# williamleif/GraphSAGE

Hardware: NVIDIA H100
Metric: seed_nodes_per_sec (higher is better)
Workload: dtype f32

## Files before the change

### graphsage_b200/_lib.py

```python
import ctypes
import os

import torch

_HERE = os.path.dirname(os.path.abspath(__file__))
LIB_PATH = os.path.join(_HERE, "csrc", "libgraphsage_b200.so")

ABI_VERSION = 2
GS_F32, GS_BF16, GS_F64 = 0, 1, 2
ACT_NONE, ACT_RELU = 0, 1
COMBINE_ADD, COMBINE_CONCAT = 0, 1
MATH_FP32_SIMT, MATH_TF32X3, MATH_TF32, MATH_BF16 = 0, 1, 2, 3
CSR_MEAN, CSR_MEAN_SELF, CSR_MAX = 0, 1, 2
MAX_SEGMENTS = 4

c_i32, c_i64, c_u64, c_vp = ctypes.c_int32, ctypes.c_int64, ctypes.c_uint64, ctypes.c_void_p


class Segment(ctypes.Structure):
    _fields_ = [("self_ids", c_vp), ("neigh_ids", c_vp), ("self_row0", c_i64), ("neigh_row0", c_i64),
                ("n", c_i64), ("k", c_i32), ("_pad", c_i32), ("out_row0", c_i64)]


MAX_SHARDS = 16


class ShardedTable(ctypes.Structure):
    _fields_ = [("base", c_vp * MAX_SHARDS), ("row_start", c_i64 * (MAX_SHARDS + 1)), ("n_shards", c_i32),
                ("my_shard", c_i32), ("n_global_rows", c_i64), ("zero_row", c_i64), ("remap", c_vp)]


class GemmPart(ctypes.Structure):
    _fields_ = [("A", c_vp), ("lda", c_i64), ("K", c_i32), ("B", c_vp), ("ldb", c_i64), ("N", c_i32)]


class RowRange(ctypes.Structure):
    _fields_ = [("ids", c_vp), ("row0", c_i64), ("n", c_i64)]


class GemmRowIds(ctypes.Structure):
    _fields_ = [("n_table_rows", c_i64), ("n_ranges", c_i32), ("_pad", c_i32), ("ranges", RowRange * MAX_SEGMENTS)]


MAX_EMBED_LISTS = 8
MAX_UNIQUE_SAMPLED = 1024
UNIQUE_DRAW_BUDGET = 1 << 20
WALK_MAX_WALKS = 1 << 20
WALK_MAX_LEN = 33


class EmbedGradList(ctypes.Structure):
    _fields_ = [("ids", c_vp), ("grad", c_vp), ("ldg", c_i64), ("n", c_i64), ("group", c_i32), ("scale", ctypes.c_float)]


class DropoutSite(ctypes.Structure):
    _fields_ = [("seed", c_u64), ("call", ctypes.c_uint32), ("rate", ctypes.c_float), ("call_dev", c_vp)]


_SIGNATURES = {
    "gs_version": (c_i32, []),
    "gs_last_error_string": (ctypes.c_char_p, []),
    "gs_set_tuning": (c_i32, [ctypes.c_char_p, c_i32]),
    "gs_sample_padded": (c_i32, [c_vp, c_i64, c_i32, c_vp, c_i64, c_i32, c_vp, c_u64, c_u64, c_vp, c_vp, c_vp]),
    "gs_sample_padded_khop": (c_i32, [c_vp, c_i64, c_i32, c_vp, c_i64, ctypes.POINTER(c_i32), c_i32, c_u64, c_u64, c_vp,
                                      ctypes.POINTER(c_vp), c_vp]),
    "gs_build_padded_adj": (c_i32, [c_vp, c_vp, c_i64, c_i32, c_vp, c_u64, c_u64, c_vp, c_vp, c_vp]),
    "gs_sample_unigram": (c_i32, [c_vp, c_i64, c_i32, c_u64, c_u64, c_vp, c_vp, c_vp]),
    "gs_sample_unigram_unique": (c_i32, [c_vp, c_i64, c_i32, c_u64, c_u64, c_vp, c_vp, c_vp, c_vp]),
    "gs_sample_csr": (c_i32, [c_vp, c_vp, c_i64, c_vp, c_i64, c_i32, c_i32, c_u64, c_u64, c_vp, c_i32, c_vp, c_vp]),
    "gs_perm_prefix_host": (c_i32, [c_u64, c_u64, c_i32, c_i32, ctypes.POINTER(c_i32)]),
    "gs_gather_rows": (c_i32, [c_vp, c_i32, c_i64, c_i32, c_i64, c_vp, c_i64, c_vp, c_i64, c_vp]),
    "gs_gather_mean": (c_i32, [c_vp, c_i32, c_i64, c_i32, c_i64, ctypes.POINTER(Segment), c_i32, c_i32, c_vp, c_vp,
                               c_i64, c_vp]),
    "gs_gather_mean_sharded": (c_i32, [ctypes.POINTER(ShardedTable), c_i32, c_i32, c_i64, ctypes.POINTER(Segment), c_i32,
                                       c_i32, c_i32, c_vp, c_vp, c_vp, c_i64, c_vp]),
    "gs_halo_begin": (c_i32, [c_vp, c_i64, c_vp, c_vp]),
    "gs_halo_claim": (c_i32, [ctypes.POINTER(ShardedTable), c_vp, c_i64, c_vp, c_vp, c_vp, c_i64, c_vp]),
    "gs_halo_fetch": (c_i32, [ctypes.POINTER(ShardedTable), c_i32, c_i64, c_vp, c_vp, c_i64, c_vp, c_i64, c_vp]),
    "gs_halo_translate": (c_i32, [ctypes.POINTER(ShardedTable), c_vp, c_i64, c_vp, c_vp, c_vp]),
    "gs_translate_ids": (c_i32, [ctypes.POINTER(ShardedTable), c_vp, c_i64, c_vp, c_vp]),
    "gs_gather_rows_sharded": (c_i32, [ctypes.POINTER(ShardedTable), c_i32, c_i32, c_i64, c_vp, c_i64, c_vp, c_i64, c_vp]),
    "gs_shard_alloc": (c_i32, [c_i64, ctypes.POINTER(c_vp)]),
    "gs_shard_free": (c_i32, [c_vp]),
    "gs_ipc_export": (c_i32, [c_vp, ctypes.c_char_p]),
    "gs_ipc_import": (c_i32, [ctypes.c_char_p, ctypes.POINTER(c_vp)]),
    "gs_ipc_close": (c_i32, [c_vp]),
    "gs_gather_rows_f32": (c_i32, [c_vp, c_i32, c_i64, c_i32, c_i64, c_vp, c_i64, c_i64, c_vp, c_i64, c_vp]),
    "gs_cast_rows_bf16": (c_i32, [c_vp, c_i64, c_i32, c_i64, c_vp, c_i64, c_vp]),
    "gs_rmat_degrees": (c_i32, [c_i32, c_i64, ctypes.c_double, ctypes.c_double, ctypes.c_double, ctypes.c_double,
                                ctypes.c_double, c_u64, c_u64, c_u64, c_u64, c_vp, c_vp]),
    "gs_rmat_fill": (c_i32, [c_i32, c_i64, ctypes.c_double, ctypes.c_double, ctypes.c_double, ctypes.c_double, c_u64, c_u64,
                             c_u64, c_u64, c_vp, c_vp, c_vp, c_i64, c_i64, c_vp]),
    "gs_segment_max": (c_i32, [c_vp, c_i64, c_i32, c_i32, c_i64, c_vp, c_i64, c_vp]),
    "gs_sage_gemm_workspace_bytes": (c_i64, [c_i64, ctypes.POINTER(GemmPart), c_i32, c_i32]),
    "gs_sage_gemm": (c_i32, [c_i64, ctypes.POINTER(GemmPart), c_i32, c_i32, c_vp, c_i32, c_i32, c_vp, c_i64, c_vp,
                             c_vp]),
    "gs_sage_gemm_pack": (c_i32, [ctypes.POINTER(GemmPart), c_i32, c_i32, c_vp, c_vp]),
    "gs_sage_gemm_prepacked": (c_i32, [c_i64, ctypes.POINTER(GemmPart), c_i32, c_i32, c_vp, c_i32, c_i32, c_vp, c_i64,
                                       c_vp, c_vp]),
    "gs_sage_gemm_rows": (c_i32, [c_i64, ctypes.POINTER(GemmPart), ctypes.POINTER(GemmRowIds), c_i32, c_i32, c_vp, c_i32, c_i32,
                                  c_vp, c_i64, c_vp, c_vp]),
    "gs_gather_mean_img_bytes": (c_i64, [c_i64, c_i32, c_i32]),
    "gs_gather_mean_img": (c_i32, [c_vp, c_i64, ctypes.POINTER(ShardedTable), c_i32, c_vp, c_i32, c_i64, ctypes.POINTER(Segment),
                                   c_i32, c_i32, c_i32, c_vp, c_vp]),
    "gs_sage_gemm_img": (c_i32, [c_i64, ctypes.POINTER(GemmPart), c_i32, c_i32, c_vp, c_i32, c_vp, c_i64, c_vp, c_vp, c_i32,
                                 c_vp]),
    "gs_sage_layer_small": (c_i32, [c_vp, c_i64, c_i32, c_i64, ctypes.POINTER(Segment), c_i32, ctypes.POINTER(GemmPart),
                                    c_i32, c_i32, c_vp, c_i32, c_i32, c_vp, c_i64, c_vp, c_u64, c_vp]),
    "gs_maxpool_mlp_workspace_bytes": (c_i64, [c_i32, c_i32]),
    "gs_maxpool_mlp_pack": (c_i32, [c_vp, c_i64, c_i32, c_i32, c_vp, c_vp]),
    "gs_maxpool_mlp_fused": (c_i32, [c_vp, c_i64, c_i32, c_i64, c_vp, c_i64, c_i64, c_i32, c_vp, c_vp, c_i32, c_vp, c_i64,
                                     c_vp]),
    "gs_meanpool_mlp_fused": (c_i32, [c_vp, c_i64, c_i32, c_i64, c_vp, c_i64, c_i64, c_i32, c_vp, c_vp, c_i32, c_vp, c_i64,
                                      c_vp]),
    "gs_pool_mlp_dp_bytes": (c_i64, [c_i64, c_i32, c_i32]),
    "gs_pool_mlp_backward_dp": (c_i32, [c_vp, c_i64, c_i32, c_i64, c_vp, c_i64, c_i64, c_i32, c_vp, c_vp, c_i32, c_vp, c_i64,
                                        c_i32, c_vp, c_vp]),
    "gs_pool_mlp_dw_workspace_bytes": (c_i64, [c_i64, c_i32, c_i32, c_i32]),
    "gs_pool_mlp_backward_dw": (c_i32, [c_vp, c_i64, c_i32, c_i64, c_vp, c_i64, c_i64, c_i32, c_i32, c_vp, c_vp, c_i64, c_vp,
                                        c_i64, c_vp, c_vp]),
    "gs_pool_mlp_dx_pack_bytes": (c_i64, [c_i32, c_i32]),
    "gs_pool_mlp_dx_pack": (c_i32, [c_vp, c_i64, c_i32, c_i32, c_vp, c_vp]),
    "gs_pool_mlp_backward_dx": (c_i32, [c_i64, c_i32, c_i32, c_vp, c_vp, c_i32, c_vp, c_i64, c_vp]),
    "gs_pipeline_step": (c_i32, [c_vp, c_vp, c_i64, ctypes.POINTER(c_vp), c_i32, c_vp, c_vp, c_i64, c_vp, c_vp, c_vp, c_vp,
                                 c_vp, c_vp]),
    "gs_l2_normalize_rows": (c_i32, [c_vp, c_i64, c_i32, c_i64, c_vp]),
    "gs_bump_counter": (c_i32, [c_vp, c_u64, c_vp]),
    "gs_embedding_grad_workspace_bytes": (c_i64, [ctypes.POINTER(EmbedGradList), c_i32, c_i64, c_i32]),
    "gs_embedding_grad": (c_i32, [ctypes.POINTER(EmbedGradList), c_i32, c_i64, c_i32, c_vp, c_i64, c_vp, c_i64, c_vp]),
    "gs_gather_mean_dropout": (c_i32, [c_vp, c_i64, c_i32, c_i64, ctypes.POINTER(Segment), c_i32, ctypes.POINTER(DropoutSite),
                                       ctypes.POINTER(DropoutSite), c_i32, c_vp, c_vp, c_i64, c_vp]),
    "gs_dropout_apply": (c_i32, [c_vp, c_i64, c_i64, c_i32, c_i32, ctypes.c_float, DropoutSite, c_i32, c_vp, c_i64, c_vp]),
    "gs_embedding_grad_dropout": (c_i32, [ctypes.POINTER(EmbedGradList), ctypes.POINTER(DropoutSite), c_i32, c_i64, c_i32, c_vp,
                                          c_i64, c_vp, c_i64, c_vp]),
    "gs_embedding_sgd": (c_i32, [ctypes.POINTER(EmbedGradList), c_i32, c_i64, c_i32, ctypes.c_float, c_vp, c_i64, c_vp, c_i64,
                                 c_vp]),
    "gs_seq_lengths": (c_i32, [c_vp, c_i64, c_i64, c_i32, c_i32, c_vp, c_vp]),
    "gs_lstm_forward": (c_i32, [c_vp, c_i64, c_vp, c_i64, c_vp, c_i64, c_i32, c_i32, c_vp, c_i64, c_vp, c_i64, c_vp, c_i64,
                                c_vp, c_i64, c_vp]),
    "gs_lstm_backward": (c_i32, [c_vp, c_i64, c_vp, c_i64, c_vp, c_i64, c_vp, c_vp, c_i64, c_i64, c_i32, c_i32, c_vp, c_i64,
                                 c_vp]),
    "gs_skipgram_workspace_bytes": (c_i64, [c_i64, c_i32, c_i32]),
    "gs_skipgram_grad": (c_i32, [c_vp, c_i64, c_vp, c_i64, c_i64, c_i32, c_vp, c_vp, c_i64, c_vp, c_i32, c_vp, c_vp, c_vp, c_vp,
                                 c_i64, c_vp, c_vp, c_i64, c_vp, c_i64, c_vp]),
    "gs_sgd_orders": (c_i32, [c_vp, c_i32, c_i64, c_i32, c_vp, c_vp]),
    "gs_sgd_fit": (c_i32, [c_vp, c_i32, c_i64, c_i32, c_i64, c_vp, c_i64, c_vp, c_i32, c_i32, ctypes.c_double, ctypes.c_double,
                           c_vp, c_i64, c_vp, c_vp]),
    "gs_random_walks_workspace_bytes": (c_i64, [c_i64, c_i32, c_i32]),
    "gs_random_walks": (c_i32, [c_vp, c_vp, c_i64, c_vp, c_i64, c_i32, c_i32, c_u64, c_u64, c_i64, c_vp, c_i64, c_vp, c_vp]),
    "gs_random_walks_emit": (c_i32, [c_vp, c_i64, c_i32, c_i32, c_vp, c_i64, c_vp, c_vp]),
    "gs_csr_aggregate": (c_i32, [c_vp, c_i32, c_i64, c_i32, c_i64, c_vp, c_vp, c_i64, c_vp, c_i64, c_i32, c_vp, c_i64, c_vp]),
}

_lib = None


def lib():
    global _lib
    if _lib is None:
        if not os.path.exists(LIB_PATH):
            raise ImportError(
                "graphsage_b200: %s is missing - build it with `python -m graphsage_b200.build` "
                "(there is no CPU fallback)" % LIB_PATH)
        _lib = ctypes.CDLL(LIB_PATH)
        for name, (res, args) in _SIGNATURES.items():
            fn = getattr(_lib, name)
            fn.restype, fn.argtypes = res, args
        if _lib.gs_version() != ABI_VERSION:
            raise ImportError("graphsage_b200: %s has ABI version %d, this binding needs %d - rebuild it"
                              % (LIB_PATH, _lib.gs_version(), ABI_VERSION))
        for kv in os.environ.get("GS_TUNING", "").split(","):
            if "=" in kv:
                k, v = kv.split("=", 1)
                _lib.gs_set_tuning(k.strip().encode(), int(v))
    return _lib


def exported_symbols():
    return sorted(_SIGNATURES)


def check(rc):
    if rc != 0:
        msg = lib().gs_last_error_string().decode("utf-8", "replace")
        raise RuntimeError("libgraphsage_b200 error %d: %s" % (rc, msg))


def stream_ptr():
    return torch.cuda.current_stream().cuda_stream


def ptr(t):
    return 0 if t is None else t.data_ptr()


def require_cuda(*tensors):
    for t in tensors:
        if t is not None and not t.is_cuda:
            raise RuntimeError("graphsage_b200: tensor on %s - the hot path is CUDA-only (no CPU fallback)" % t.device)


def set_tuning(key, value):
    return lib().gs_set_tuning(key.encode(), int(value))


def perm_prefix_host(seed, counter, max_deg, k):
    buf = (c_i32 * max(k, 1))()
    check(lib().gs_perm_prefix_host(seed & (2**64 - 1), counter & (2**64 - 1), max_deg, k, buf))
    return list(buf[:k])
```

### graphsage_b200/csrc/gather.cu

```cuda
#include "common.cuh"

namespace gs {

struct SegTable {
  gs_segment s[GS_MAX_SEGMENTS];
  int32_t n_segments;
  int64_t total_rows;
};

__device__ __forceinline__ int find_segment(const SegTable& t, int64_t r, int64_t& local) {
  int si = 0;
  int64_t base = 0, end = 0;
#pragma unroll
  for (int q = 0; q < GS_MAX_SEGMENTS - 1; ++q) {
    if (q < t.n_segments - 1) {
      end += t.s[q].n;
      if (r >= end) {
        base = end;
        si = q + 1;
      }
    }
  }
  local = r - base;
  return si;
}

__device__ __forceinline__ int64_t clamp_row(int64_t id, int64_t n_rows) {
  return (id < 0 || id >= n_rows) ? n_rows - 1 : id;
}

__device__ __forceinline__ float4 mask_tail(float4 v, int col0, int F) {
  if (col0 + 1 >= F) v.y = 0.f;
  if (col0 + 2 >= F) v.z = 0.f;
  if (col0 + 3 >= F) v.w = 0.f;
  return v;
}

template <int kUnroll>
__global__ void __launch_bounds__(256) gather_mean_ldg_kernel(const float* __restrict__ src, int64_t n_src_rows, int F,
                                                              int64_t pitch, const __grid_constant__ SegTable tab, int include_self,
                                                              float* __restrict__ out_self,
                                                              float* __restrict__ out_mean, int64_t out_pitch) {
  const int ncol4 = (int)(out_pitch >> 2);
  for (int64_t r = blockIdx.x; r < tab.total_rows; r += gridDim.x) {
    int64_t i;
    const gs_segment& sg = tab.s[find_segment(tab, r, i)];
    const int k = sg.k;
    const int64_t orow = sg.out_row0 + i;
    const int64_t srow = clamp_row(sg.self_ids ? (int64_t)sg.self_ids[i] : sg.self_row0 + i, n_src_rows);
    for (int c = threadIdx.x; c < ncol4; c += blockDim.x) {
      const int col0 = c * 4;
      float4 acc = make_float4(0.f, 0.f, 0.f, 0.f);
      float4 sv = acc;
      if (col0 < F) {
        int j = 0;
        for (; j + kUnroll <= k; j += kUnroll) {
          float4 v[kUnroll];
#pragma unroll
          for (int u = 0; u < kUnroll; ++u) {
            int64_t nr = clamp_row(sg.neigh_ids ? (int64_t)sg.neigh_ids[i * k + j + u] : sg.neigh_row0 + i * k + j + u,
                                   n_src_rows);
            v[u] = ldg_nc_f4(reinterpret_cast<const float4*>(src + nr * pitch) + c);
          }
#pragma unroll
          for (int u = 0; u < kUnroll; ++u) {
            acc.x += v[u].x; acc.y += v[u].y; acc.z += v[u].z; acc.w += v[u].w;
          }
        }
        for (; j < k; ++j) {
          int64_t nr = clamp_row(sg.neigh_ids ? (int64_t)sg.neigh_ids[i * k + j] : sg.neigh_row0 + i * k + j, n_src_rows);
          float4 v = ldg_nc_f4(reinterpret_cast<const float4*>(src + nr * pitch) + c);
          acc.x += v.x; acc.y += v.y; acc.z += v.z; acc.w += v.w;
        }
        if (include_self || out_self) sv = ldg_nc_f4(reinterpret_cast<const float4*>(src + srow * pitch) + c);
        float div = (float)(k + (include_self ? 1 : 0));
        if (include_self) { acc.x += sv.x; acc.y += sv.y; acc.z += sv.z; acc.w += sv.w; }
        acc.x /= div; acc.y /= div; acc.z /= div; acc.w /= div;
        acc = mask_tail(acc, col0, F);
        sv = mask_tail(sv, col0, F);
      }
      reinterpret_cast<float4*>(out_mean + orow * out_pitch)[c] = acc;
      if (out_self) reinterpret_cast<float4*>(out_self + orow * out_pitch)[c] = sv;
    }
  }
}

struct DropTab {
  DropSite neigh[GS_MAX_SEGMENTS];
  DropSite self[GS_MAX_SEGMENTS];
};

template <bool kDrop>
__global__ void __launch_bounds__(256) gather_mean_scalar_kernel(const float* __restrict__ src, int64_t n_src_rows, int F,
                                                                 int64_t pitch, const __grid_constant__ SegTable tab, int include_self,
                                                                 float* __restrict__ out_self,
                                                                 float* __restrict__ out_mean, int64_t out_pitch,
                                                                 const __grid_constant__ DropTab drop) {
  __shared__ uint32_t drop_off[2 * GS_MAX_SEGMENTS];
  if constexpr (kDrop) {
    if (threadIdx.x < 2 * GS_MAX_SEGMENTS) {
      const int s = threadIdx.x % GS_MAX_SEGMENTS;
      drop_off[threadIdx.x] = drop_call_offset(threadIdx.x < GS_MAX_SEGMENTS ? drop.neigh[s] : drop.self[s]);
    }
    __syncthreads();
  }
  for (int64_t r = blockIdx.x; r < tab.total_rows; r += gridDim.x) {
    int64_t i;
    const int si = find_segment(tab, r, i);
    const gs_segment& sg = tab.s[si];
    const int k = sg.k;
    const int64_t orow = sg.out_row0 + i;
    const int64_t srow = clamp_row(sg.self_ids ? (int64_t)sg.self_ids[i] : sg.self_row0 + i, n_src_rows);
    DropSite nsite{}, ssite{};
    if constexpr (kDrop) {
      nsite = with_call_offset(drop.neigh[si], drop_off[si]);
      ssite = with_call_offset(drop.self[si], drop_off[GS_MAX_SEGMENTS + si]);
    }
    for (int c = threadIdx.x; c < (int)out_pitch; c += blockDim.x) {
      float acc = 0.f, sv = 0.f;
      if (c < F) {
        for (int j = 0; j < k; ++j) {
          int64_t nr = clamp_row(sg.neigh_ids ? (int64_t)sg.neigh_ids[i * k + j] : sg.neigh_row0 + i * k + j, n_src_rows);
          if constexpr (kDrop) acc += drop_col(nsite, i * k + j, c, src[nr * pitch + c]);
          else acc += src[nr * pitch + c];
        }
        sv = src[srow * pitch + c];
        if constexpr (kDrop) sv = drop_col(ssite, i, c, sv);
        if (include_self) acc += sv;
        acc /= (float)(k + (include_self ? 1 : 0));
      }
      out_mean[orow * out_pitch + c] = acc;
      if (out_self) out_self[orow * out_pitch + c] = sv;
    }
  }
}

__global__ void __launch_bounds__(192) gather_mean_tma_kernel(const float* __restrict__ src, int64_t n_src_rows, int F,
                                                              int64_t pitch, const __grid_constant__ SegTable tab, int include_self,
                                                              float* __restrict__ out_self,
                                                              float* __restrict__ out_mean, int64_t out_pitch,
                                                              int row_bytes) {
  extern __shared__ __align__(128) unsigned char smem[];
  __shared__ __align__(8) uint64_t bar;
  if (threadIdx.x == 0) {
    mbar_init(&bar, 1);
    fence_mbar_init();
  }
  __syncthreads();
  const int ncol4 = (int)(out_pitch >> 2);
  const int row_f4 = row_bytes >> 4;
  uint32_t phase = 0;
  for (int64_t r = blockIdx.x; r < tab.total_rows; r += gridDim.x) {
    int64_t i;
    const gs_segment& sg = tab.s[find_segment(tab, r, i)];
    const int k = sg.k;
    const int64_t orow = sg.out_row0 + i;
    if (threadIdx.x < 32) {
      if (threadIdx.x == 0) mbar_expect_tx(&bar, (uint32_t)((k + 1) * row_bytes));
      __syncwarp();
      for (int j = threadIdx.x; j <= k; j += 32) {
        int64_t id;
        if (j < k) id = sg.neigh_ids ? (int64_t)sg.neigh_ids[i * k + j] : sg.neigh_row0 + i * k + j;
        else id = sg.self_ids ? (int64_t)sg.self_ids[i] : sg.self_row0 + i;
        id = clamp_row(id, n_src_rows);
        bulk_g2s(smem + (size_t)j * row_bytes, src + id * pitch, (uint32_t)row_bytes, &bar);
      }
    }
    mbar_wait(&bar, phase);
    phase ^= 1u;
    const float4* rows = reinterpret_cast<const float4*>(smem);
    for (int c = threadIdx.x; c < ncol4; c += blockDim.x) {
      const int col0 = c * 4;
      float4 acc = make_float4(0.f, 0.f, 0.f, 0.f);
      float4 sv = acc;
      if (col0 < F) {
#pragma unroll 5
        for (int j = 0; j < k; ++j) {
          float4 v = rows[j * row_f4 + c];
          acc.x += v.x; acc.y += v.y; acc.z += v.z; acc.w += v.w;
        }
        sv = rows[k * row_f4 + c];
        float div = (float)(k + (include_self ? 1 : 0));
        if (include_self) { acc.x += sv.x; acc.y += sv.y; acc.z += sv.z; acc.w += sv.w; }
        acc.x /= div; acc.y /= div; acc.z /= div; acc.w /= div;
        acc = mask_tail(acc, col0, F);
        sv = mask_tail(sv, col0, F);
      }
      reinterpret_cast<float4*>(out_mean + orow * out_pitch)[c] = acc;
      if (out_self) reinterpret_cast<float4*>(out_self + orow * out_pitch)[c] = sv;
    }
    __syncthreads();
  }
}

struct DenseRows {
  const float* src;
  int64_t n_rows, pitch;
  __device__ __forceinline__ const float* row(int64_t id) const { return src + clamp_row(id, n_rows) * pitch; }
};

struct ShardTab {
  const float* base[GS_MAX_SHARDS];
  int64_t row_start[GS_MAX_SHARDS + 1];
  int32_t n_shards, my_shard;
  int64_t n_global_rows;
  int64_t zero_row;
  const int32_t* remap;
};

struct ShardRows {
  ShardTab t;
  int64_t pitch;
  int32_t locators;
  const float* staging;
  __device__ __forceinline__ const float* row(int64_t id) const {
    const float* mine = t.base[t.my_shard];
    if (locators) {
      if (id >= 0) return mine + id * pitch;
      if (locators == 2) return staging + (-id - 1) * pitch;
      id = -id - 1;
    } else if (id < 0 || id >= t.n_global_rows - 1) {
      return mine + t.zero_row * pitch;
    } else if (t.remap) {
      const int32_t s = __ldg(t.remap + id);
      if (s >= 0) return mine + (int64_t)s * pitch;
    } else if (id >= t.row_start[t.my_shard] && id < t.row_start[t.my_shard + 1]) {
      return mine + (id - t.row_start[t.my_shard]) * pitch;
    }
    int o = 0;
#pragma unroll
    for (int q = 1; q < GS_MAX_SHARDS; ++q)
      if (q < t.n_shards && id >= t.row_start[q]) o = q;
    return t.base[o] + (id - t.row_start[o]) * pitch;
  }
};

constexpr int kGroupRows = 13;

struct GatherImg {
  unsigned char* base;
  int32_t kblocks, n_mtiles;
  int32_t want_self;
};

__device__ __forceinline__ void gather_img_store(const GatherImg& im, int part, int64_t orow, int c, float4 v) {
  const int kb = c >> 3, chunk = c & 7;
  const int64_t mt = orow >> 7;
  const int r = (int)(orow & 127);
  unsigned char* dst = im.base + ((((int64_t)part * im.n_mtiles + mt) * im.kblocks + kb) * 2) * 16384 +
                       (uint32_t)(r * 128 + ((chunk ^ (r & 7)) << 4));
  uint4 hi, lo;
  hi.x = __float_as_uint(v.x) & 0xFFFFE000u; hi.y = __float_as_uint(v.y) & 0xFFFFE000u;
  hi.z = __float_as_uint(v.z) & 0xFFFFE000u; hi.w = __float_as_uint(v.w) & 0xFFFFE000u;
  lo.x = __float_as_uint(v.x - __uint_as_float(hi.x)) & 0xFFFFE000u; lo.y = __float_as_uint(v.y - __uint_as_float(hi.y)) & 0xFFFFE000u;
  lo.z = __float_as_uint(v.z - __uint_as_float(hi.z)) & 0xFFFFE000u; lo.w = __float_as_uint(v.w - __uint_as_float(hi.w)) & 0xFFFFE000u;
  *reinterpret_cast<uint4*>(dst) = hi;
  *reinterpret_cast<uint4*>(dst + 16384) = lo;
}

template <class Rows, bool kDrop>
__global__ void __launch_bounds__(192, 3) gather_mean_tma2_kernel(const __grid_constant__ Rows rows_of, int F,
                                                               const __grid_constant__ SegTable tab,
                                                               int include_self, float* __restrict__ out_self,
                                                               float* __restrict__ out_mean, int64_t out_pitch,
                                                               int row_bytes, const __grid_constant__ GatherImg img,
                                                               const __grid_constant__ DropTab drop) {
  extern __shared__ __align__(128) unsigned char smem[];
  __shared__ __align__(8) uint64_t bar[2];
  __shared__ uint32_t drop_off[2 * GS_MAX_SEGMENTS];
  if (threadIdx.x == 0) {
    mbar_init(&bar[0], 1);
    mbar_init(&bar[1], 1);
    fence_mbar_init();
  }
  if constexpr (kDrop) {
    if (threadIdx.x < 2 * GS_MAX_SEGMENTS) {
      const int s = threadIdx.x % GS_MAX_SEGMENTS;
      drop_off[threadIdx.x] = drop_call_offset(threadIdx.x < GS_MAX_SEGMENTS ? drop.neigh[s] : drop.self[s]);
    }
  }
  __syncthreads();
  const int ncol4 = (int)(out_pitch >> 2);
  const int row_f4 = row_bytes >> 4;
  const size_t buf_bytes = (size_t)kGroupRows * row_bytes;
  const int self_rows = (include_self || out_self || (img.base && img.want_self)) ? 1 : 0;

  int64_t r_issue = blockIdx.x;
  int g_issue = 0;
  auto issue = [&](int buf) -> bool {
    if (r_issue >= tab.total_rows) return false;
    int64_t i;
    const gs_segment& sg = tab.s[find_segment(tab, r_issue, i)];
    const int k = sg.k;
    const int rows_total = k + self_rows;
    const int first = g_issue * kGroupRows;
    const int cnt = min(kGroupRows, rows_total - first);
    if (threadIdx.x < 32) {
      if (threadIdx.x == 0) mbar_expect_tx(&bar[buf], (uint32_t)(cnt * row_bytes));
      __syncwarp();
      for (int j = threadIdx.x; j < cnt; j += 32) {
        const int jj = first + j;
        int64_t id;
        if (jj < k) id = sg.neigh_ids ? (int64_t)sg.neigh_ids[i * k + jj] : sg.neigh_row0 + i * k + jj;
        else id = sg.self_ids ? (int64_t)sg.self_ids[i] : sg.self_row0 + i;
        bulk_g2s(smem + buf * buf_bytes + (size_t)j * row_bytes, rows_of.row(id), (uint32_t)row_bytes, &bar[buf]);
      }
    }
    if (first + cnt >= rows_total) { r_issue += gridDim.x; g_issue = 0; } else { ++g_issue; }
    return true;
  };

  uint32_t phase[2] = {0u, 0u};
  int buf = 0;
  bool have = issue(0);
  int64_t r = blockIdx.x;
  int g = 0;
  float4 acc[2];
  acc[0] = acc[1] = make_float4(0.f, 0.f, 0.f, 0.f);
  while (have) {
    const bool have_next = issue(buf ^ 1);
    int64_t i;
    const int si = find_segment(tab, r, i);
    const gs_segment& sg = tab.s[si];
    const int k = sg.k;
    const int rows_total = k + self_rows;
    const int first = g * kGroupRows;
    const int cnt = min(kGroupRows, rows_total - first);
    const bool last = first + cnt >= rows_total;
    mbar_wait(&bar[buf], phase[buf]);
    phase[buf] ^= 1u;
    const float4* rows = reinterpret_cast<const float4*>(smem + buf * buf_bytes);
    const int nn = last ? cnt - self_rows : cnt;
    DropSite nsite{};
    if constexpr (kDrop) nsite = with_call_offset(drop.neigh[si], drop_off[si]);
#pragma unroll
    for (int q = 0; q < 2; ++q) {
      const int c = threadIdx.x + q * blockDim.x;
      if (c < ncol4 && c * 4 < F) {
        float4 a = acc[q];
        for (int j = 0; j < nn; ++j) {
          float4 v = rows[j * row_f4 + c];
          if constexpr (kDrop) v = drop4(nsite, i * k + first + j, (uint32_t)c, v);
          a.x += v.x; a.y += v.y; a.z += v.z; a.w += v.w;
        }
        acc[q] = a;
      }
    }
    if (last) {
      const int64_t orow = sg.out_row0 + i;
      const int ncol_img = img.base ? img.kblocks * 8 : 0;
#pragma unroll
      for (int q = 0; q < 2; ++q) {
        const int c = threadIdx.x + q * blockDim.x;
        if (c < ncol4 || c < ncol_img) {
          float4 a = make_float4(0.f, 0.f, 0.f, 0.f), sv = a;
          if (c < ncol4 && c * 4 < F) {
            a = acc[q];
            if (self_rows) {
              sv = rows[(cnt - 1) * row_f4 + c];
              if constexpr (kDrop) sv = drop4(with_call_offset(drop.self[si], drop_off[GS_MAX_SEGMENTS + si]), i, (uint32_t)c, sv);
            }
            const float div = (float)(k + (include_self ? 1 : 0));
            if (include_self) { a.x += sv.x; a.y += sv.y; a.z += sv.z; a.w += sv.w; }
            a.x /= div; a.y /= div; a.z /= div; a.w /= div;
            a = mask_tail(a, c * 4, F);
            sv = mask_tail(sv, c * 4, F);
          }
          if (c < ncol4) {
            if (out_mean) reinterpret_cast<float4*>(out_mean + orow * out_pitch)[c] = a;
            if (out_self) reinterpret_cast<float4*>(out_self + orow * out_pitch)[c] = sv;
          }
          if (c < ncol_img) {
            if (img.want_self) gather_img_store(img, 0, orow, c, sv);
            gather_img_store(img, img.want_self ? 1 : 0, orow, c, a);
          }
          if (c < ncol4) acc[q] = make_float4(0.f, 0.f, 0.f, 0.f);
        }
      }
      r += gridDim.x;
      g = 0;
    } else {
      ++g;
    }
    __syncthreads();
    buf ^= 1;
    have = have_next;
  }
}

__global__ void __launch_bounds__(192) gather_mean_bf16_tma2_kernel(const uint16_t* __restrict__ src, int64_t n_src_rows, int F,
                                                                    int64_t pitch, const __grid_constant__ SegTable tab,
                                                                    int include_self, float* __restrict__ out_self,
                                                                    float* __restrict__ out_mean, int64_t out_pitch,
                                                                    int row_bytes) {
  extern __shared__ __align__(128) unsigned char smem[];
  __shared__ __align__(8) uint64_t bar[2];
  if (threadIdx.x == 0) {
    mbar_init(&bar[0], 1);
    mbar_init(&bar[1], 1);
    fence_mbar_init();
  }
  __syncthreads();
  const int ncol8 = (int)(out_pitch >> 3);
  const int row_u4 = row_bytes >> 4;
  const size_t buf_bytes = (size_t)kGroupRows * row_bytes;
  int64_t r_issue = blockIdx.x;
  int g_issue = 0;
  auto issue = [&](int buf) -> bool {
    if (r_issue >= tab.total_rows) return false;
    int64_t i;
    const gs_segment& sg = tab.s[find_segment(tab, r_issue, i)];
    const int k = sg.k;
    const int rows_total = k + 1;
    const int first = g_issue * kGroupRows;
    const int cnt = min(kGroupRows, rows_total - first);
    if (threadIdx.x < 32) {
      if (threadIdx.x == 0) mbar_expect_tx(&bar[buf], (uint32_t)(cnt * row_bytes));
      __syncwarp();
      for (int j = threadIdx.x; j < cnt; j += 32) {
        const int jj = first + j;
        int64_t id;
        if (jj < k) id = sg.neigh_ids ? (int64_t)sg.neigh_ids[i * k + jj] : sg.neigh_row0 + i * k + jj;
        else id = sg.self_ids ? (int64_t)sg.self_ids[i] : sg.self_row0 + i;
        id = clamp_row(id, n_src_rows);
        bulk_g2s(smem + buf * buf_bytes + (size_t)j * row_bytes, src + id * pitch, (uint32_t)row_bytes, &bar[buf]);
      }
    }
    if (first + cnt >= rows_total) { r_issue += gridDim.x; g_issue = 0; } else { ++g_issue; }
    return true;
  };
  auto widen = [](uint4 u, float (&v)[8]) {
    const uint32_t w[4] = {u.x, u.y, u.z, u.w};
#pragma unroll
    for (int e = 0; e < 4; ++e) {
      v[2 * e] = __uint_as_float(w[e] << 16);
      v[2 * e + 1] = __uint_as_float(w[e] & 0xffff0000u);
    }
  };
  uint32_t phase[2] = {0u, 0u};
  int buf = 0;
  bool have = issue(0);
  int64_t r = blockIdx.x;
  int g = 0;
  float acc[8];
#pragma unroll
  for (int e = 0; e < 8; ++e) acc[e] = 0.f;
  const int c = threadIdx.x;
  while (have) {
    const bool have_next = issue(buf ^ 1);
    int64_t i;
    const gs_segment& sg = tab.s[find_segment(tab, r, i)];
    const int k = sg.k;
    const int rows_total = k + 1;
    const int first = g * kGroupRows;
    const int cnt = min(kGroupRows, rows_total - first);
    const bool last = first + cnt >= rows_total;
    mbar_wait(&bar[buf], phase[buf]);
    phase[buf] ^= 1u;
    const uint4* rows = reinterpret_cast<const uint4*>(smem + buf * buf_bytes);
    const int nn = last ? cnt - 1 : cnt;
    if (c < ncol8 && c * 8 < F) {
      for (int j = 0; j < nn; ++j) {
        float v[8];
        widen(rows[j * row_u4 + c], v);
#pragma unroll
        for (int e = 0; e < 8; ++e) acc[e] += v[e];
      }
    }
    if (last) {
      const int64_t orow = sg.out_row0 + i;
      if (c < ncol8) {
        float a[8], sv[8];
#pragma unroll
        for (int e = 0; e < 8; ++e) { a[e] = 0.f; sv[e] = 0.f; }
        if (c * 8 < F) {
          widen(rows[(cnt - 1) * row_u4 + c], sv);
          const float div = (float)(k + (include_self ? 1 : 0));
#pragma unroll
          for (int e = 0; e < 8; ++e) {
            float t = acc[e];
            if (include_self) t += sv[e];
            a[e] = (c * 8 + e < F) ? t / div : 0.f;
            if (c * 8 + e >= F) sv[e] = 0.f;
          }
        }
        float4* om = reinterpret_cast<float4*>(out_mean + orow * out_pitch) + 2 * c;
        om[0] = make_float4(a[0], a[1], a[2], a[3]);
        om[1] = make_float4(a[4], a[5], a[6], a[7]);
        if (out_self) {
          float4* os = reinterpret_cast<float4*>(out_self + orow * out_pitch) + 2 * c;
          os[0] = make_float4(sv[0], sv[1], sv[2], sv[3]);
          os[1] = make_float4(sv[4], sv[5], sv[6], sv[7]);
        }
#pragma unroll
        for (int e = 0; e < 8; ++e) acc[e] = 0.f;
      }
      r += gridDim.x;
      g = 0;
    } else {
      ++g;
    }
    __syncthreads();
    buf ^= 1;
    have = have_next;
  }
}

__global__ void __launch_bounds__(32) gather_rows_tma_kernel(const unsigned char* __restrict__ src, int64_t n_rows,
                                                             int64_t pitch_bytes, const int32_t* __restrict__ ids,
                                                             int64_t n, unsigned char* __restrict__ out,
                                                             int64_t out_pitch_bytes, int row_bytes) {
  extern __shared__ __align__(128) unsigned char smem[];
  __shared__ __align__(8) uint64_t bar;
  const int lane = threadIdx.x;
  if (lane == 0) {
    mbar_init(&bar, 1);
    fence_mbar_init();
  }
  __syncwarp();
  uint32_t phase = 0;
  for (int64_t base = (int64_t)blockIdx.x * 32; base < n; base += (int64_t)gridDim.x * 32) {
    int cnt = (int)((n - base) < 32 ? (n - base) : 32);
    if (lane == 0) mbar_expect_tx(&bar, (uint32_t)(cnt * row_bytes));
    __syncwarp();
    if (lane < cnt) {
      int64_t id = clamp_row(ids[base + lane], n_rows);
      bulk_g2s(smem + (size_t)lane * row_bytes, src + id * pitch_bytes, (uint32_t)row_bytes, &bar);
    }
    mbar_wait(&bar, phase);
    phase ^= 1u;
    if (lane < cnt) bulk_s2g(out + (base + lane) * out_pitch_bytes, smem + (size_t)lane * row_bytes, (uint32_t)row_bytes);
    bulk_commit();
    bulk_wait_read<0>();
    __syncwarp();
  }
  bulk_wait<0>();
}

template <typename T>
__global__ void __launch_bounds__(256) gather_rows_simple_kernel(const T* __restrict__ src, int64_t n_rows, int F,
                                                                 int64_t pitch, const int32_t* __restrict__ ids,
                                                                 int64_t n, T* __restrict__ out, int64_t out_pitch) {
  const int lane = threadIdx.x & 31;
  const int64_t warp = ((int64_t)blockIdx.x * blockDim.x + threadIdx.x) >> 5;
  const int64_t nwarps = ((int64_t)gridDim.x * blockDim.x) >> 5;
  for (int64_t i = warp; i < n; i += nwarps) {
    int64_t id = clamp_row(ids[i], n_rows);
    for (int c = lane; c < F; c += 32) out[i * out_pitch + c] = src[id * pitch + c];
  }
}

template <typename T>
__global__ void __launch_bounds__(256) gather_rows_to_f32_kernel(const T* __restrict__ src, int64_t n_rows, int F,
                                                                 int64_t pitch, const int32_t* __restrict__ ids, int64_t row0,
                                                                 int64_t n, float* __restrict__ out, int64_t out_pitch) {
  const int lane = threadIdx.x & 31;
  const int64_t warp = ((int64_t)blockIdx.x * blockDim.x + threadIdx.x) >> 5;
  const int64_t nwarps = ((int64_t)gridDim.x * blockDim.x) >> 5;
  for (int64_t i = warp; i < n; i += nwarps) {
    const int64_t id = clamp_row(ids ? (int64_t)ids[i] : row0 + i, n_rows);
    for (int c = lane; c < (int)out_pitch; c += 32) {
      float v = 0.f;
      if (c < F) {
        if constexpr (sizeof(T) == 2) v = __uint_as_float(((uint32_t)src[id * pitch + c]) << 16);
        else v = src[id * pitch + c];
      }
      out[i * out_pitch + c] = v;
    }
  }
}

__global__ void __launch_bounds__(256) gather_rows_bf16_to_f32_vec_kernel(const uint16_t* __restrict__ src, int64_t n_rows, int F,
                                                                          int64_t pitch, const int32_t* __restrict__ ids,
                                                                          int64_t row0, int64_t n, float* __restrict__ out,
                                                                          int64_t out_pitch) {
  const int lane = threadIdx.x & 31;
  const int64_t warp = ((int64_t)blockIdx.x * blockDim.x + threadIdx.x) >> 5;
  const int64_t nwarps = ((int64_t)gridDim.x * blockDim.x) >> 5;
  const int chunks = (int)(out_pitch >> 3);
  for (int64_t i = warp; i < n; i += nwarps) {
    const int64_t id = clamp_row(ids ? (int64_t)ids[i] : row0 + i, n_rows);
    const uint4* rp = reinterpret_cast<const uint4*>(src + id * pitch);
    float4* op = reinterpret_cast<float4*>(out + i * out_pitch);
    for (int c = lane; c < chunks; c += 32) {
      uint4 u = make_uint4(0u, 0u, 0u, 0u);
      if (c * 8 < F) u = __ldg(rp + c);
      const uint32_t w[4] = {u.x, u.y, u.z, u.w};
      float v[8];
#pragma unroll
      for (int e = 0; e < 4; ++e) {
        v[2 * e] = (c * 8 + 2 * e < F) ? __uint_as_float(w[e] << 16) : 0.f;
        v[2 * e + 1] = (c * 8 + 2 * e + 1 < F) ? __uint_as_float(w[e] & 0xffff0000u) : 0.f;
      }
      op[2 * c] = make_float4(v[0], v[1], v[2], v[3]);
      op[2 * c + 1] = make_float4(v[4], v[5], v[6], v[7]);
    }
  }
}

__device__ __forceinline__ uint32_t f32_to_bf16_rne(float x) {
  const uint32_t u = __float_as_uint(x);
  if ((u & 0x7fffffffu) > 0x7f800000u) return (u >> 16) | 0x40u;
  return (u + 0x7fffu + ((u >> 16) & 1u)) >> 16;
}

__global__ void __launch_bounds__(256) cast_rows_bf16_kernel(const float* __restrict__ x, int64_t n, int F, int64_t ldx,
                                                             uint16_t* __restrict__ out, int64_t out_pitch) {
  const int chunks = (int)(out_pitch >> 3);
  const int64_t total = n * chunks;
  for (int64_t q = (int64_t)blockIdx.x * blockDim.x + threadIdx.x; q < total; q += (int64_t)gridDim.x * blockDim.x) {
    const int64_t i = q / chunks;
    const int c = (int)(q - i * chunks) * 8;
    const float* xp = x + i * ldx + c;
    uint32_t h[8];
#pragma unroll
    for (int e = 0; e < 8; ++e) h[e] = (c + e < F) ? f32_to_bf16_rne(xp[e]) : 0u;
    uint4 o;
    o.x = h[0] | (h[1] << 16); o.y = h[2] | (h[3] << 16); o.z = h[4] | (h[5] << 16); o.w = h[6] | (h[7] << 16);
    *reinterpret_cast<uint4*>(out + i * out_pitch + c) = o;
  }
}

__global__ void __launch_bounds__(256) cast_rows_bf16_scalar_kernel(const float* __restrict__ x, int64_t n, int F, int64_t ldx,
                                                                    uint16_t* __restrict__ out, int64_t out_pitch) {
  const int64_t total = n * out_pitch;
  for (int64_t q = (int64_t)blockIdx.x * blockDim.x + threadIdx.x; q < total; q += (int64_t)gridDim.x * blockDim.x) {
    const int64_t i = q / out_pitch;
    const int c = (int)(q - i * out_pitch);
    out[q] = c < F ? (uint16_t)f32_to_bf16_rne(x[i * ldx + c]) : (uint16_t)0;
  }
}

__global__ void __launch_bounds__(256) dropout_apply_kernel(const float* x, int64_t ldx, int64_t rows, int F, int group,
                                                            float scale, DropSite site, int accumulate, float* out,
                                                            int64_t ldo) {
  const int nc4 = (F + 3) >> 2;
  const int64_t total = rows * nc4;
  site.call += drop_call_offset(site);
  for (int64_t q = (int64_t)blockIdx.x * blockDim.x + threadIdx.x; q < total; q += (int64_t)gridDim.x * blockDim.x) {
    const int64_t r = q / nc4;
    const int c4 = (int)(q - r * nc4);
    const u32x4 w = drop_words(site, r, (uint32_t)c4);
    const float* xr = x + (r / group) * ldx;
    float* orow = out + r * ldo;
#pragma unroll
    for (int e = 0; e < 4; ++e) {
      const int c = c4 * 4 + e;
      if (c < F) {
        const float v = pick(w, e) >= site.threshold ? (xr[c] * scale) / site.keep : 0.f;
        orow[c] = accumulate ? orow[c] + v : v;
      }
    }
  }
}

__global__ void bump_counter_kernel(unsigned long long* counter, unsigned long long inc) { *counter += inc; }

__global__ void __launch_bounds__(256) segment_max_kernel(const float* __restrict__ x, int64_t n, int k, int C,
                                                          int64_t ldx, float* __restrict__ out, int64_t ldo) {
  for (int64_t i = blockIdx.x; i < n; i += gridDim.x) {
    for (int c = threadIdx.x; c < C; c += blockDim.x) {
      float m = x[(i * k) * ldx + c];
      for (int j = 1; j < k; ++j) m = fmaxf(m, x[(i * k + j) * ldx + c]);
      out[i * ldo + c] = m;
    }
  }
}

__global__ void __launch_bounds__(256) l2_normalize_kernel(float* __restrict__ x, int64_t n, int C, int64_t ldx) {
  const int lane = threadIdx.x & 31;
  const int64_t warp = ((int64_t)blockIdx.x * blockDim.x + threadIdx.x) >> 5;
  const int64_t nwarps = ((int64_t)gridDim.x * blockDim.x) >> 5;
  for (int64_t i = warp; i < n; i += nwarps) {
    float ss = 0.f;
    for (int c = lane; c < C; c += 32) {
      float v = x[i * ldx + c];
      ss += v * v;
    }
#pragma unroll
    for (int o = 16; o > 0; o >>= 1) ss += __shfl_xor_sync(0xffffffffu, ss, o);
    float inv = 1.0f / sqrtf(fmaxf(ss, 1e-12f));
    for (int c = lane; c < C; c += 32) x[i * ldx + c] *= inv;
  }
}

__global__ void __launch_bounds__(256) translate_ids_kernel(const int32_t* __restrict__ remap, int64_t n_global_rows,
                                                            int32_t zero_row, const int32_t* __restrict__ ids, int64_t n,
                                                            int32_t* __restrict__ out) {
  for (int64_t i = (int64_t)blockIdx.x * blockDim.x + threadIdx.x; i < n; i += (int64_t)gridDim.x * blockDim.x) {
    const int32_t id = ids[i];
    int32_t loc;
    if (id < 0 || id >= n_global_rows - 1) loc = zero_row;
    else {
      loc = __ldg(remap + id);
      if (loc < 0) loc = -id - 1;
    }
    out[i] = loc;
  }
}

__device__ __forceinline__ bool halo_is_local(const ShardTab& t, int32_t id, int32_t& loc) {
  if (id < 0 || id >= t.n_global_rows - 1) { loc = (int32_t)t.zero_row; return true; }
  if (t.remap) {
    loc = __ldg(t.remap + id);
    return loc >= 0;
  }
  if (id >= t.row_start[t.my_shard] && id < t.row_start[t.my_shard + 1]) { loc = (int32_t)(id - t.row_start[t.my_shard]); return true; }
  return false;
}

__global__ void __launch_bounds__(256) halo_claim_kernel(const __grid_constant__ ShardTab t, const int32_t* __restrict__ ids,
                                                         int64_t n, int32_t* __restrict__ claim, int32_t* __restrict__ count,
                                                         int32_t* __restrict__ stage_ids, int64_t capacity) {
  for (int64_t i = (int64_t)blockIdx.x * blockDim.x + threadIdx.x; i < n; i += (int64_t)gridDim.x * blockDim.x) {
    const int32_t id = ids[i];
    int32_t loc;
    if (halo_is_local(t, id, loc)) continue;
    if (atomicCAS(claim + id, -1, -2) == -1) {
      const int32_t idx = atomicAdd(count, 1);
      if (idx < capacity) stage_ids[idx] = id;
      claim[id] = idx;
    }
  }
}

__global__ void __launch_bounds__(256) halo_translate_kernel(const __grid_constant__ ShardTab t, const int32_t* __restrict__ ids,
                                                             int64_t n, const int32_t* __restrict__ claim,
                                                             int32_t* __restrict__ out) {
  for (int64_t i = (int64_t)blockIdx.x * blockDim.x + threadIdx.x; i < n; i += (int64_t)gridDim.x * blockDim.x) {
    const int32_t id = ids[i];
    int32_t loc;
    if (!halo_is_local(t, id, loc)) loc = -claim[id] - 1;
    out[i] = loc;
  }
}

constexpr int kHaloLoads = 5;
__global__ void __launch_bounds__(256) halo_fetch_kernel(const __grid_constant__ ShardRows sr, int row_f4,
                                                         const int32_t* __restrict__ stage_ids, const int32_t* __restrict__ count,
                                                         int64_t capacity, float* __restrict__ staging, int64_t staging_pitch) {
  const int lane = threadIdx.x & 31;
  const int64_t warp = ((int64_t)blockIdx.x * blockDim.x + threadIdx.x) >> 5;
  const int64_t nwarps = ((int64_t)gridDim.x * blockDim.x) >> 5;
  int64_t n = *count;
  if (n > capacity) n = capacity;
  for (int64_t i = warp; i < n; i += nwarps) {
    const float4* src = reinterpret_cast<const float4*>(sr.row(stage_ids[i]));
    float4* dst = reinterpret_cast<float4*>(staging + i * staging_pitch);
    for (int c0 = lane; c0 < row_f4; c0 += 32 * kHaloLoads) {
      float4 v[kHaloLoads];
#pragma unroll
      for (int u = 0; u < kHaloLoads; ++u)
        if (c0 + 32 * u < row_f4) v[u] = ldg_nc_f4(src + c0 + 32 * u);
#pragma unroll
      for (int u = 0; u < kHaloLoads; ++u)
        if (c0 + 32 * u < row_f4) dst[c0 + 32 * u] = v[u];
    }
  }
}

template <int kUnroll>
__global__ void __launch_bounds__(256) gather_mean_sharded_kernel(const __grid_constant__ ShardRows st, int F,
                                                                  const __grid_constant__ SegTable tab, int include_self,
                                                                  float* __restrict__ out_self,
                                                                  float* __restrict__ out_mean, int64_t out_pitch) {
  const int ncol4 = (int)(out_pitch >> 2);
  for (int64_t r = blockIdx.x; r < tab.total_rows; r += gridDim.x) {
    int64_t i;
    const gs_segment& sg = tab.s[find_segment(tab, r, i)];
    const int k = sg.k;
    const int64_t orow = sg.out_row0 + i;
    const float* srow = st.row(sg.self_ids ? (int64_t)sg.self_ids[i] : sg.self_row0 + i);
    for (int c = threadIdx.x; c < ncol4; c += blockDim.x) {
      const int col0 = c * 4;
      float4 acc = make_float4(0.f, 0.f, 0.f, 0.f);
      float4 sv = acc;
      if (col0 < F) {
        int j = 0;
        for (; j + kUnroll <= k; j += kUnroll) {
          float4 v[kUnroll];
#pragma unroll
          for (int u = 0; u < kUnroll; ++u) {
            const float* p = st.row(sg.neigh_ids ? (int64_t)sg.neigh_ids[i * k + j + u] : sg.neigh_row0 + i * k + j + u);
            v[u] = ldg_nc_f4(reinterpret_cast<const float4*>(p) + c);
          }
#pragma unroll
          for (int u = 0; u < kUnroll; ++u) {
            acc.x += v[u].x; acc.y += v[u].y; acc.z += v[u].z; acc.w += v[u].w;
          }
        }
        for (; j < k; ++j) {
          const float* p = st.row(sg.neigh_ids ? (int64_t)sg.neigh_ids[i * k + j] : sg.neigh_row0 + i * k + j);
          float4 v = ldg_nc_f4(reinterpret_cast<const float4*>(p) + c);
          acc.x += v.x; acc.y += v.y; acc.z += v.z; acc.w += v.w;
        }
        if (include_self || out_self) sv = ldg_nc_f4(reinterpret_cast<const float4*>(srow) + c);
        float div = (float)(k + (include_self ? 1 : 0));
        if (include_self) { acc.x += sv.x; acc.y += sv.y; acc.z += sv.z; acc.w += sv.w; }
        acc.x /= div; acc.y /= div; acc.z /= div; acc.w /= div;
        acc = mask_tail(acc, col0, F);
        sv = mask_tail(sv, col0, F);
      }
      reinterpret_cast<float4*>(out_mean + orow * out_pitch)[c] = acc;
      if (out_self) reinterpret_cast<float4*>(out_self + orow * out_pitch)[c] = sv;
    }
  }
}

__global__ void __launch_bounds__(256) gather_rows_sharded_kernel(const __grid_constant__ ShardRows st, int F,
                                                                  const int32_t* __restrict__ ids, int64_t n,
                                                                  float* __restrict__ out, int64_t out_pitch) {
  const int lane = threadIdx.x & 31;
  const int64_t warp = ((int64_t)blockIdx.x * blockDim.x + threadIdx.x) >> 5;
  const int64_t nwarps = ((int64_t)gridDim.x * blockDim.x) >> 5;
  const int ncol4 = (int)(out_pitch >> 2);
  for (int64_t i = warp; i < n; i += nwarps) {
    const float* p = st.row(ids[i]);
    for (int c = lane; c < ncol4; c += 32) {
      float4 v = make_float4(0.f, 0.f, 0.f, 0.f);
      if (c * 4 < F) v = mask_tail(ldg_nc_f4(reinterpret_cast<const float4*>(p) + c), c * 4, F);
      reinterpret_cast<float4*>(out + i * out_pitch)[c] = v;
    }
  }
}

static inline bool aligned16(const void* p) { return (reinterpret_cast<uintptr_t>(p) & 15u) == 0; }

}


namespace gs {
template <class Rows, bool kDrop = false>
static int32_t launch_gather_tma2(const Rows& rows_of, int F, const SegTable& tab, int include_self, float* out_self, float* out_mean,
                                  int64_t out_pitch, const GatherImg& img, cudaStream_t st, const DropTab* drop = nullptr) {
  const int32_t rc_attr = ensure_dyn_smem((const void*)gather_mean_tma2_kernel<Rows, kDrop>, 200 * 1024);
  if (rc_attr != GS_OK) return rc_attr;
  const int ncol4 = (int)(out_pitch / 4);
  const int row_bytes = ((F + 3) / 4) * 16;
  const size_t smem2 = (size_t)2 * kGroupRows * row_bytes;
  int threads = ((ncol4 + 31) / 32) * 32;
  if (threads > 160) threads = 160;
  if (threads < 32) threads = 32;
  int per_sm = (int)((224 * 1024) / (smem2 + 1024));
  if (per_sm < 1) per_sm = 1;
  int lim = tuning("gather_ctas_per_sm", 8);
  if (per_sm > lim) per_sm = lim;
  int64_t blocks = tab.total_rows;
  int64_t cap = (int64_t)sm_count() * per_sm;
  if (blocks > cap) blocks = cap;
  DropTab no_drop;
  memset(&no_drop, 0, sizeof(no_drop));
  gather_mean_tma2_kernel<Rows, kDrop><<<(unsigned)blocks, threads, smem2, st>>>(rows_of, F, tab, include_self, out_self,
                                                                                 out_mean, out_pitch, row_bytes, img,
                                                                                 drop ? *drop : no_drop);
  return launch_check("gather_mean_tma2_kernel");
}
}

extern "C" {

int32_t gs_gather_rows(const void* feats, int32_t dtype, int64_t n_rows, int32_t F, int64_t pitch, const int32_t* ids,
                       int64_t n, void* out, int64_t out_pitch, void* stream) {
  GS_REQUIRE(n >= 0 && F >= 0, "gs_gather_rows: negative size");
  if (n == 0 || F == 0) return GS_OK;
  GS_REQUIRE(feats && ids && out, "gs_gather_rows: NULL pointer");
  GS_REQUIRE(dtype == GS_F32 || dtype == GS_BF16, "gs_gather_rows: dtype %d", dtype);
  GS_REQUIRE(n_rows > 0 && pitch >= F && out_pitch >= F, "gs_gather_rows: pitch < F");
  const int es = dtype == GS_F32 ? 4 : 2;
  cudaStream_t st = (cudaStream_t)stream;
  const int row_bytes = ((F * es + 15) / 16) * 16;
  const bool tma_ok = gs::aligned16(feats) && gs::aligned16(out) && (pitch * es) % 16 == 0 && (out_pitch * es) % 16 == 0 &&
                      row_bytes <= pitch * es && row_bytes <= out_pitch * es && row_bytes * 32 <= 200 * 1024;
  if (tma_ok && gs::tuning("gather_variant", 2) != 0) {
    size_t smem = (size_t)row_bytes * 32;
    {
      const int32_t rc_attr = gs::ensure_dyn_smem((const void*)gs::gather_rows_tma_kernel, 200 * 1024);
      if (rc_attr != GS_OK) return rc_attr;
    }
    int per_sm = (int)((220 * 1024) / (smem + 1024));
    if (per_sm < 1) per_sm = 1;
    if (per_sm > 16) per_sm = 16;
    int64_t blocks = (n + 31) / 32;
    int64_t cap = (int64_t)gs::sm_count() * per_sm;
    if (blocks > cap) blocks = cap;
    gs::gather_rows_tma_kernel<<<(unsigned)blocks, 32, smem, st>>>((const unsigned char*)feats, n_rows, pitch * es, ids, n,
                                                                   (unsigned char*)out, out_pitch * es, row_bytes);
    return gs::launch_check("gather_rows_tma_kernel");
  }
  int64_t blocks = (n + 7) / 8;
  int64_t cap = (int64_t)gs::sm_count() * 8;
  if (blocks > cap) blocks = cap;
  if (dtype == GS_F32)
    gs::gather_rows_simple_kernel<float><<<(unsigned)blocks, 256, 0, st>>>((const float*)feats, n_rows, F, pitch, ids, n,
                                                                           (float*)out, out_pitch);
  else
    gs::gather_rows_simple_kernel<uint16_t><<<(unsigned)blocks, 256, 0, st>>>((const uint16_t*)feats, n_rows, F, pitch, ids,
                                                                              n, (uint16_t*)out, out_pitch);
  return gs::launch_check("gather_rows_simple_kernel");
}

int32_t gs_gather_mean(const void* src, int32_t dtype, int64_t n_src_rows, int32_t F, int64_t pitch,
                       const gs_segment* segments_host, int32_t n_segments, int32_t include_self, void* out_self,
                       void* out_mean, int64_t out_pitch, void* stream) {
  GS_REQUIRE(dtype == GS_F32 || dtype == GS_BF16, "gs_gather_mean: dtype %d (GS_F32 or GS_BF16)", dtype);
  GS_REQUIRE(n_segments >= 0 && n_segments <= GS_MAX_SEGMENTS, "gs_gather_mean: n_segments=%d (max %d)", n_segments,
             GS_MAX_SEGMENTS);
  GS_REQUIRE(segments_host || n_segments == 0, "gs_gather_mean: segments_host is NULL");
  gs::SegTable tab;
  memset(&tab, 0, sizeof(tab));
  tab.n_segments = n_segments;
  int kmax = 0;
  for (int s = 0; s < n_segments; ++s) {
    tab.s[s] = segments_host[s];
    GS_REQUIRE(tab.s[s].n >= 0 && tab.s[s].k >= 1, "gs_gather_mean: segment %d has n=%lld k=%d", s, (long long)tab.s[s].n,
               tab.s[s].k);
    tab.total_rows += tab.s[s].n;
    if (tab.s[s].k > kmax) kmax = tab.s[s].k;
  }
  if (tab.total_rows == 0) return GS_OK;
  GS_REQUIRE(src && out_mean, "gs_gather_mean: NULL pointer");
  GS_REQUIRE(F > 0 && pitch >= F && out_pitch >= F && n_src_rows > 0, "gs_gather_mean: bad F/pitch");
  cudaStream_t st = (cudaStream_t)stream;
  if (dtype == GS_BF16) {
    const int64_t f8 = ((int64_t)F + 7) / 8 * 8;
    if (!(gs::aligned16(src) && gs::aligned16(out_mean) && (!out_self || gs::aligned16(out_self)) && pitch % 8 == 0 &&
          out_pitch % 8 == 0 && f8 <= pitch && f8 <= out_pitch && f8 / 8 <= 192)) {
      gs::set_error("gs_gather_mean(GS_BF16): needs 16-byte aligned rows (pitch %% 8 == 0), out_pitch %% 8 == 0 and F <= 1536");
      return GS_ERR_UNSUPPORTED;
    }
    const int32_t rc_attr = gs::ensure_dyn_smem((const void*)gs::gather_mean_bf16_tma2_kernel, 200 * 1024);
    if (rc_attr != GS_OK) return rc_attr;
    const int row_bytes = (int)(f8 * 2);
    const size_t smem2 = (size_t)2 * gs::kGroupRows * row_bytes;
    const int ncol8 = (int)(out_pitch / 8);
    int threads = ((ncol8 + 31) / 32) * 32;
    if (threads < 32) threads = 32;
    GS_REQUIRE(threads <= 192, "gs_gather_mean(GS_BF16): out_pitch too wide");
    int per_sm = (int)((224 * 1024) / (smem2 + 1024));
    if (per_sm < 1) per_sm = 1;
    int lim = gs::tuning("gather_ctas_per_sm", 8);
    if (per_sm > lim) per_sm = lim;
    int64_t blocks = tab.total_rows;
    int64_t cap = (int64_t)gs::sm_count() * per_sm;
    if (blocks > cap) blocks = cap;
    gs::gather_mean_bf16_tma2_kernel<<<(unsigned)blocks, threads, smem2, st>>>((const uint16_t*)src, n_src_rows, F, pitch, tab,
                                                                              include_self, (float*)out_self, (float*)out_mean,
                                                                              out_pitch, row_bytes);
    return gs::launch_check("gather_mean_bf16_tma2_kernel");
  }
  const float* fsrc = (const float*)src;
  const bool vec_ok = gs::aligned16(src) && gs::aligned16(out_mean) && (!out_self || gs::aligned16(out_self)) &&
                      pitch % 4 == 0 && out_pitch % 4 == 0 && ((F + 3) / 4) * 4 <= pitch;
  if (!vec_ok) {
    int64_t blocks = tab.total_rows;
    int64_t cap = (int64_t)gs::sm_count() * 8;
    if (blocks > cap) blocks = cap;
    gs::DropTab no_drop;
    memset(&no_drop, 0, sizeof(no_drop));
    gs::gather_mean_scalar_kernel<false><<<(unsigned)blocks, 256, 0, st>>>(fsrc, n_src_rows, F, pitch, tab, include_self,
                                                                           (float*)out_self, (float*)out_mean, out_pitch,
                                                                           no_drop);
    return gs::launch_check("gather_mean_scalar_kernel");
  }
  const int ncol4 = (int)(out_pitch / 4);
  const int row_bytes = ((F + 3) / 4) * 16;
  const size_t smem = (size_t)row_bytes * (kmax + 1);
  const int variant = gs::tuning("gather_variant", 2);
  if (variant == 2 && ncol4 <= 2 * 160) {
    const gs::DenseRows rows_of{fsrc, n_src_rows, pitch};
    gs::GatherImg img;
    memset(&img, 0, sizeof(img));
    return gs::launch_gather_tma2(rows_of, F, tab, include_self, (float*)out_self, (float*)out_mean, out_pitch, img, st);
  }
  if (variant >= 1 && smem <= 200 * 1024) {
    {
      const int32_t rc_attr = gs::ensure_dyn_smem((const void*)gs::gather_mean_tma_kernel, 200 * 1024);
      if (rc_attr != GS_OK) return rc_attr;
    }
    int threads = ((ncol4 + 31) / 32) * 32;
    if (threads > 192) threads = 192;
    if (threads < 32) threads = 32;
    int per_sm = (int)((224 * 1024) / (smem + 1024));
    if (per_sm < 1) per_sm = 1;
    int lim = gs::tuning("gather_ctas_per_sm", 8);
    if (per_sm > lim) per_sm = lim;
    int64_t blocks = tab.total_rows;
    int64_t cap = (int64_t)gs::sm_count() * per_sm;
    if (blocks > cap) blocks = cap;
    gs::gather_mean_tma_kernel<<<(unsigned)blocks, threads, smem, st>>>(fsrc, n_src_rows, F, pitch, tab, include_self,
                                                                        (float*)out_self, (float*)out_mean, out_pitch,
                                                                        row_bytes);
    return gs::launch_check("gather_mean_tma_kernel");
  }
  int threads = ((ncol4 + 31) / 32) * 32;
  if (threads > 256) threads = 256;
  int64_t blocks = tab.total_rows;
  int64_t cap = (int64_t)gs::sm_count() * gs::tuning("gather_ctas_per_sm", 8);
  if (blocks > cap) blocks = cap;
  gs::gather_mean_ldg_kernel<5><<<(unsigned)blocks, threads, 0, st>>>(fsrc, n_src_rows, F, pitch, tab, include_self,
                                                                      (float*)out_self, (float*)out_mean, out_pitch);
  return gs::launch_check("gather_mean_ldg_kernel");
}

int32_t gs_gather_rows_f32(const void* feats, int32_t dtype, int64_t n_rows, int32_t F, int64_t pitch, const int32_t* ids,
                           int64_t row0, int64_t n, float* out, int64_t out_pitch, void* stream) {
  GS_REQUIRE(n >= 0 && F >= 0, "gs_gather_rows_f32: negative size");
  if (n == 0 || out_pitch == 0) return GS_OK;
  GS_REQUIRE(feats && out, "gs_gather_rows_f32: NULL pointer");
  GS_REQUIRE(dtype == GS_F32 || dtype == GS_BF16, "gs_gather_rows_f32: dtype %d", dtype);
  GS_REQUIRE(n_rows > 0 && pitch >= F && out_pitch >= F, "gs_gather_rows_f32: pitch < F");
  int64_t blocks = (n + 7) / 8;
  int64_t cap = (int64_t)gs::sm_count() * 8;
  if (blocks > cap) blocks = cap;
  if (dtype == GS_F32)
    gs::gather_rows_to_f32_kernel<float><<<(unsigned)blocks, 256, 0, (cudaStream_t)stream>>>(
        (const float*)feats, n_rows, F, pitch, ids, row0, n, out, out_pitch);
  else if (pitch % 8 == 0 && out_pitch % 8 == 0 && gs::aligned16(feats) && gs::aligned16(out) && out_pitch <= pitch)
    gs::gather_rows_bf16_to_f32_vec_kernel<<<(unsigned)blocks, 256, 0, (cudaStream_t)stream>>>(
        (const uint16_t*)feats, n_rows, F, pitch, ids, row0, n, out, out_pitch);
  else
    gs::gather_rows_to_f32_kernel<uint16_t><<<(unsigned)blocks, 256, 0, (cudaStream_t)stream>>>(
        (const uint16_t*)feats, n_rows, F, pitch, ids, row0, n, out, out_pitch);
  return gs::launch_check("gather_rows_to_f32_kernel");
}

int32_t gs_cast_rows_bf16(const float* x, int64_t n, int32_t F, int64_t ldx, void* out_bf16, int64_t out_pitch,
                          void* stream) {
  GS_REQUIRE(n >= 0 && F >= 0 && ldx >= F && out_pitch >= F, "gs_cast_rows_bf16: bad sizes");
  if (n == 0 || out_pitch == 0) return GS_OK;
  GS_REQUIRE(x && out_bf16, "gs_cast_rows_bf16: NULL pointer");
  const bool vec = out_pitch % 8 == 0 && gs::aligned16(out_bf16) && ldx >= ((F + 7) / 8) * 8;
  int64_t blocks = ((vec ? n * (out_pitch / 8) : n * out_pitch) + 255) / 256;
  int64_t cap = (int64_t)gs::sm_count() * 8;
  if (blocks > cap) blocks = cap;
  if (vec)
    gs::cast_rows_bf16_kernel<<<(unsigned)blocks, 256, 0, (cudaStream_t)stream>>>(x, n, F, ldx, (uint16_t*)out_bf16, out_pitch);
  else
    gs::cast_rows_bf16_scalar_kernel<<<(unsigned)blocks, 256, 0, (cudaStream_t)stream>>>(x, n, F, ldx, (uint16_t*)out_bf16,
                                                                                         out_pitch);
  return gs::launch_check("cast_rows_bf16_kernel");
}

int32_t gs_bump_counter(uint64_t* counter_dev, uint64_t inc, void* stream) {
  GS_REQUIRE(counter_dev != nullptr, "gs_bump_counter: NULL counter");
  gs::bump_counter_kernel<<<1, 1, 0, (cudaStream_t)stream>>>((unsigned long long*)counter_dev, (unsigned long long)inc);
  return gs::launch_check("bump_counter_kernel");
}

int32_t gs_segment_max(const float* x, int64_t n, int32_t k, int32_t C, int64_t ldx, float* out, int64_t ldo,
                       void* stream) {
  GS_REQUIRE(n >= 0 && k >= 1 && C >= 0, "gs_segment_max: bad sizes");
  if (n == 0 || C == 0) return GS_OK;
  GS_REQUIRE(x && out, "gs_segment_max: NULL pointer");
  int64_t blocks = n;
  int64_t cap = (int64_t)gs::sm_count() * 8;
  if (blocks > cap) blocks = cap;
  gs::segment_max_kernel<<<(unsigned)blocks, 256, 0, (cudaStream_t)stream>>>(x, n, k, C, ldx, out, ldo);
  return gs::launch_check("segment_max_kernel");
}

static int32_t check_site(const gs_dropout_site& s, const char* who) {
  GS_REQUIRE(s.rate >= 0.f && s.rate < 1.f, "%s: dropout rate %g outside [0, 1)", who, (double)s.rate);
  return GS_OK;
}

int32_t gs_gather_mean_dropout(const float* src, int64_t n_src_rows, int32_t F, int64_t pitch, const gs_segment* segments_host,
                               int32_t n_segments, const gs_dropout_site* neigh_sites_host,
                               const gs_dropout_site* self_sites_host, int32_t include_self, float* out_self,
                               float* out_mean, int64_t out_pitch, void* stream) {
  GS_REQUIRE(n_segments >= 0 && n_segments <= GS_MAX_SEGMENTS, "gs_gather_mean_dropout: n_segments=%d (max %d)", n_segments,
             GS_MAX_SEGMENTS);
  GS_REQUIRE((segments_host && neigh_sites_host && self_sites_host) || n_segments == 0,
             "gs_gather_mean_dropout: segments / sites are NULL");
  gs::SegTable tab;
  memset(&tab, 0, sizeof(tab));
  gs::DropTab drop;
  memset(&drop, 0, sizeof(drop));
  tab.n_segments = n_segments;
  for (int s = 0; s < n_segments; ++s) {
    tab.s[s] = segments_host[s];
    GS_REQUIRE(tab.s[s].n >= 0 && tab.s[s].k >= 1, "gs_gather_mean_dropout: segment %d has n=%lld k=%d", s,
               (long long)tab.s[s].n, tab.s[s].k);
    int32_t rc = check_site(neigh_sites_host[s], "gs_gather_mean_dropout");
    if (rc == GS_OK) rc = check_site(self_sites_host[s], "gs_gather_mean_dropout");
    if (rc != GS_OK) return rc;
    drop.neigh[s] = gs::make_drop_site(neigh_sites_host[s]);
    drop.self[s] = gs::make_drop_site(self_sites_host[s]);
    tab.total_rows += tab.s[s].n;
  }
  if (tab.total_rows == 0) return GS_OK;
  GS_REQUIRE(src && out_mean, "gs_gather_mean_dropout: NULL pointer");
  GS_REQUIRE(F > 0 && pitch >= F && out_pitch >= F && n_src_rows > 0, "gs_gather_mean_dropout: bad F/pitch");
  cudaStream_t st = (cudaStream_t)stream;
  const int ncol4 = (int)(out_pitch / 4);
  const bool vec_ok = gs::aligned16(src) && gs::aligned16(out_mean) && (!out_self || gs::aligned16(out_self)) &&
                      pitch % 4 == 0 && out_pitch % 4 == 0 && ((F + 3) / 4) * 4 <= pitch;
  if (vec_ok && ncol4 <= 2 * 160) {
    const gs::DenseRows rows_of{src, n_src_rows, pitch};
    gs::GatherImg img;
    memset(&img, 0, sizeof(img));
    return gs::launch_gather_tma2<gs::DenseRows, true>(rows_of, F, tab, include_self, out_self, out_mean, out_pitch, img, st,
                                                       &drop);
  }
  int64_t blocks = tab.total_rows;
  int64_t cap = (int64_t)gs::sm_count() * 8;
  if (blocks > cap) blocks = cap;
  gs::gather_mean_scalar_kernel<true><<<(unsigned)blocks, 256, 0, st>>>(src, n_src_rows, F, pitch, tab, include_self, out_self,
                                                                        out_mean, out_pitch, drop);
  return gs::launch_check("gather_mean_scalar_kernel<drop>");
}

int32_t gs_dropout_apply(const float* x, int64_t ldx, int64_t rows, int32_t F, int32_t group, float scale,
                         gs_dropout_site site, int32_t accumulate, float* out, int64_t ldo, void* stream) {
  int32_t rc = check_site(site, "gs_dropout_apply");
  if (rc != GS_OK) return rc;
  GS_REQUIRE(rows >= 0 && F >= 0 && group >= 1, "gs_dropout_apply: bad sizes (rows=%lld F=%d group=%d)", (long long)rows, F,
             group);
  if (rows == 0 || F == 0) return GS_OK;
  GS_REQUIRE(x && out, "gs_dropout_apply: NULL pointer");
  GS_REQUIRE(ldx >= F && ldo >= F, "gs_dropout_apply: row stride < F");
  GS_REQUIRE(x != out || (group == 1 && ldx == ldo), "gs_dropout_apply: in place needs group == 1 and ldo == ldx");
  const int64_t total = rows * ((F + 3) / 4);
  int64_t blocks = (total + 255) / 256;
  int64_t cap = (int64_t)gs::sm_count() * 16;
  if (blocks > cap) blocks = cap;
  gs::dropout_apply_kernel<<<(unsigned)blocks, 256, 0, (cudaStream_t)stream>>>(x, ldx, rows, F, group, scale,
                                                                                gs::make_drop_site(site), accumulate, out, ldo);
  return gs::launch_check("dropout_apply_kernel");
}

int32_t gs_l2_normalize_rows(float* x, int64_t n, int32_t C, int64_t ldx, void* stream) {
  GS_REQUIRE(n >= 0 && C >= 0, "gs_l2_normalize_rows: bad sizes");
  if (n == 0 || C == 0) return GS_OK;
  GS_REQUIRE(x, "gs_l2_normalize_rows: NULL pointer");
  int64_t blocks = (n + 7) / 8;
  int64_t cap = (int64_t)gs::sm_count() * 8;
  if (blocks > cap) blocks = cap;
  gs::l2_normalize_kernel<<<(unsigned)blocks, 256, 0, (cudaStream_t)stream>>>(x, n, C, ldx);
  return gs::launch_check("l2_normalize_kernel");
}

}

static int32_t fill_shard_tab(const gs_sharded_table* t, gs::ShardRows& sr, int64_t pitch, const char* who) {
  GS_REQUIRE(t != nullptr, "%s: table is NULL", who);
  GS_REQUIRE(t->n_shards >= 1 && t->n_shards <= GS_MAX_SHARDS, "%s: n_shards=%d (max %d)", who, t->n_shards, GS_MAX_SHARDS);
  GS_REQUIRE(t->my_shard >= 0 && t->my_shard < t->n_shards, "%s: my_shard=%d", who, t->my_shard);
  GS_REQUIRE(t->n_global_rows > 0 && t->row_start[0] == 0 && t->row_start[t->n_shards] == t->n_global_rows - 1,
             "%s: row_start must run from 0 to n_global_rows - 1", who);
  for (int i = 0; i < t->n_shards; ++i)
    GS_REQUIRE(t->row_start[i] <= t->row_start[i + 1], "%s: row_start must be non-decreasing (shard %d)", who, i);
  GS_REQUIRE(t->zero_row >= 0, "%s: zero_row < 0", who);
  GS_REQUIRE(pitch % 4 == 0, "%s: pitch must be a multiple of 4 floats", who);
  memset(&sr, 0, sizeof(sr));
  gs::ShardTab& st = sr.t;
  for (int i = 0; i < t->n_shards; ++i) {
    GS_REQUIRE(t->base[i] != nullptr && gs::aligned16(t->base[i]), "%s: shard %d pointer NULL or not 16-byte aligned", who, i);
    st.base[i] = (const float*)t->base[i];
  }
  for (int i = 0; i <= t->n_shards; ++i) st.row_start[i] = t->row_start[i];
  for (int i = t->n_shards + 1; i <= GS_MAX_SHARDS; ++i) st.row_start[i] = t->row_start[t->n_shards];
  st.n_shards = t->n_shards;
  st.my_shard = t->my_shard;
  st.n_global_rows = t->n_global_rows;
  st.zero_row = t->zero_row;
  st.remap = t->remap;
  sr.pitch = pitch;
  return GS_OK;
}

extern "C" {

int32_t gs_translate_ids(const gs_sharded_table* table_host, const int32_t* ids, int64_t n, int32_t* out, void* stream) {
  GS_REQUIRE(table_host && table_host->remap, "gs_translate_ids: the table has no remap (no replicas)");
  GS_REQUIRE(n >= 0, "gs_translate_ids: n < 0");
  if (n == 0) return GS_OK;
  GS_REQUIRE(ids && out, "gs_translate_ids: NULL pointer");
  GS_REQUIRE(table_host->zero_row >= 0 && table_host->zero_row < 0x7fffffffLL, "gs_translate_ids: zero_row out of range");
  int64_t blocks = (n + 255) / 256;
  int64_t cap = (int64_t)gs::sm_count() * 8;
  if (blocks > cap) blocks = cap;
  gs::translate_ids_kernel<<<(unsigned)blocks, 256, 0, (cudaStream_t)stream>>>(table_host->remap, table_host->n_global_rows,
                                                                                (int32_t)table_host->zero_row, ids, n, out);
  return gs::launch_check("translate_ids_kernel");
}

int64_t gs_gather_mean_img_bytes(int64_t rows, int32_t F, int32_t want_self) {
  if (rows < 0 || F < 1) return -1;
  const int64_t n_mtiles = (rows + 127) / 128, kblocks = (F + 31) / 32;
  return (want_self ? 2 : 1) * n_mtiles * kblocks * 2 * 16384;
}

int32_t gs_gather_mean_img(const void* src, int64_t n_src_rows, const gs_sharded_table* table_host, int32_t ids_are_locators,
                           const void* staging, int32_t F, int64_t pitch, const gs_segment* segments_host, int32_t n_segments,
                           int32_t include_self, int32_t want_self, void* images, void* stream) {
  GS_REQUIRE((src != nullptr) != (table_host != nullptr), "gs_gather_mean_img: pass either a dense table or a sharded one");
  GS_REQUIRE(n_segments >= 0 && n_segments <= GS_MAX_SEGMENTS && (segments_host || n_segments == 0),
             "gs_gather_mean_img: bad segments");
  gs::SegTable tab;
  memset(&tab, 0, sizeof(tab));
  tab.n_segments = n_segments;
  int64_t rows = 0;
  for (int s = 0; s < n_segments; ++s) {
    tab.s[s] = segments_host[s];
    GS_REQUIRE(tab.s[s].n >= 0 && tab.s[s].k >= 1, "gs_gather_mean_img: segment %d has n=%lld k=%d", s, (long long)tab.s[s].n,
               tab.s[s].k);
    tab.total_rows += tab.s[s].n;
    if (tab.s[s].out_row0 + tab.s[s].n > rows) rows = tab.s[s].out_row0 + tab.s[s].n;
  }
  if (tab.total_rows == 0) return GS_OK;
  GS_REQUIRE(images && (reinterpret_cast<uintptr_t>(images) & 1023u) == 0, "gs_gather_mean_img: images must be 1024-byte aligned");
  const int64_t out_pitch = ((int64_t)F + 7) / 8 * 8;
  const int ncol4 = (int)(out_pitch / 4);
  if (ncol4 > 2 * 160 || F < 1 || pitch % 4 != 0 || pitch < ((F + 3) / 4) * 4 || gs::tuning("gather_variant", 2) != 2) {
    gs::set_error("gs_gather_mean_img: needs F <= 1280, 16-byte row pitch and the bulk-copy gather (F=%d pitch=%lld)", F, (long long)pitch);
    return GS_ERR_UNSUPPORTED;
  }
  gs::GatherImg img;
  img.base = (unsigned char*)images;
  img.kblocks = (F + 31) / 32;
  img.n_mtiles = (int32_t)((rows + 127) / 128);
  img.want_self = want_self ? 1 : 0;
  if (src) {
    GS_REQUIRE(gs::aligned16(src) && n_src_rows > 0, "gs_gather_mean_img: table must be 16-byte aligned");
    const gs::DenseRows rows_of{(const float*)src, n_src_rows, pitch};
    return gs::launch_gather_tma2(rows_of, F, tab, include_self, nullptr, nullptr, out_pitch, img, (cudaStream_t)stream);
  }
  gs::ShardRows sr;
  int32_t rc = fill_shard_tab(table_host, sr, pitch, "gs_gather_mean_img");
  if (rc != GS_OK) return rc;
  GS_REQUIRE(ids_are_locators >= 0 && ids_are_locators <= 2 && (ids_are_locators != 2 || staging != nullptr),
             "gs_gather_mean_img: ids_are_locators = 2 needs the staging buffer");
  sr.locators = ids_are_locators;
  sr.staging = (const float*)staging;
  return gs::launch_gather_tma2(sr, F, tab, include_self, nullptr, nullptr, out_pitch, img, (cudaStream_t)stream);
}

int32_t gs_halo_begin(int32_t* claim, int64_t n_global_rows, int32_t* count, void* stream) {
  GS_REQUIRE(claim && count && n_global_rows > 0, "gs_halo_begin: bad arguments");
  GS_CUDA(cudaMemsetAsync(claim, 0xff, (size_t)n_global_rows * 4, (cudaStream_t)stream));
  GS_CUDA(cudaMemsetAsync(count, 0, 4, (cudaStream_t)stream));
  return GS_OK;
}

int32_t gs_halo_claim(const gs_sharded_table* table_host, const int32_t* ids, int64_t n, int32_t* claim, int32_t* count,
                      int32_t* stage_ids, int64_t capacity, void* stream) {
  gs::ShardRows sr;
  int32_t rc = fill_shard_tab(table_host, sr, 4, "gs_halo_claim");
  if (rc != GS_OK) return rc;
  GS_REQUIRE(n >= 0 && capacity >= 0, "gs_halo_claim: negative size");
  if (n == 0) return GS_OK;
  GS_REQUIRE(ids && claim && count && stage_ids, "gs_halo_claim: NULL pointer");
  int64_t blocks = (n + 255) / 256;
  int64_t cap = (int64_t)gs::sm_count() * 8;
  if (blocks > cap) blocks = cap;
  gs::halo_claim_kernel<<<(unsigned)blocks, 256, 0, (cudaStream_t)stream>>>(sr.t, ids, n, claim, count, stage_ids, capacity);
  return gs::launch_check("halo_claim_kernel");
}

int32_t gs_halo_translate(const gs_sharded_table* table_host, const int32_t* ids, int64_t n, const int32_t* claim, int32_t* out,
                          void* stream) {
  gs::ShardRows sr;
  int32_t rc = fill_shard_tab(table_host, sr, 4, "gs_halo_translate");
  if (rc != GS_OK) return rc;
  GS_REQUIRE(n >= 0, "gs_halo_translate: n < 0");
  if (n == 0) return GS_OK;
  GS_REQUIRE(ids && claim && out, "gs_halo_translate: NULL pointer");
  int64_t blocks = (n + 255) / 256;
  int64_t cap = (int64_t)gs::sm_count() * 8;
  if (blocks > cap) blocks = cap;
  gs::halo_translate_kernel<<<(unsigned)blocks, 256, 0, (cudaStream_t)stream>>>(sr.t, ids, n, claim, out);
  return gs::launch_check("halo_translate_kernel");
}

int32_t gs_halo_fetch(const gs_sharded_table* table_host, int32_t F, int64_t pitch, const int32_t* stage_ids,
                      const int32_t* count, int64_t capacity, float* staging, int64_t staging_pitch, void* stream) {
  gs::ShardRows sr;
  int32_t rc = fill_shard_tab(table_host, sr, pitch, "gs_halo_fetch");
  if (rc != GS_OK) return rc;
  if (capacity == 0) return GS_OK;
  GS_REQUIRE(stage_ids && count && staging && gs::aligned16(staging) && staging_pitch % 4 == 0 && F > 0 &&
                 pitch >= ((F + 3) / 4) * 4 && staging_pitch >= ((F + 3) / 4) * 4,
             "gs_halo_fetch: bad arguments");
  sr.locators = 0;
  sr.staging = nullptr;
  sr.t.remap = nullptr;
  const int blocks = gs::sm_count() * gs::tuning("halo_fetch_ctas_per_sm", 2);
  gs::halo_fetch_kernel<<<(unsigned)blocks, 256, 0, (cudaStream_t)stream>>>(sr, (F + 3) / 4, stage_ids, count, capacity, staging,
                                                                            staging_pitch);
  return gs::launch_check("halo_fetch_kernel");
}

int32_t gs_gather_mean_sharded(const gs_sharded_table* table_host, int32_t dtype, int32_t F, int64_t pitch,
                               const gs_segment* segments_host, int32_t n_segments, int32_t include_self,
                               int32_t ids_are_locators, const void* staging, void* out_self, void* out_mean,
                               int64_t out_pitch, void* stream) {
  GS_REQUIRE(dtype == GS_F32, "gs_gather_mean_sharded: only GS_F32 (dtype=%d)", dtype);
  GS_REQUIRE(n_segments >= 0 && n_segments <= GS_MAX_SEGMENTS && (segments_host || n_segments == 0),
             "gs_gather_mean_sharded: bad segments");
  gs::ShardRows sr;
  int32_t rc = fill_shard_tab(table_host, sr, pitch, "gs_gather_mean_sharded");
  if (rc != GS_OK) return rc;
  GS_REQUIRE(ids_are_locators >= 0 && ids_are_locators <= 2 && (ids_are_locators != 2 || staging != nullptr),
             "gs_gather_mean_sharded: ids_are_locators = 2 needs the staging buffer");
  sr.locators = ids_are_locators;
  sr.staging = (const float*)staging;
  gs::SegTable tab;
  memset(&tab, 0, sizeof(tab));
  tab.n_segments = n_segments;
  for (int s = 0; s < n_segments; ++s) {
    tab.s[s] = segments_host[s];
    GS_REQUIRE(tab.s[s].n >= 0 && tab.s[s].k >= 1, "gs_gather_mean_sharded: segment %d has n=%lld k=%d", s,
               (long long)tab.s[s].n, tab.s[s].k);
    tab.total_rows += tab.s[s].n;
  }
  if (tab.total_rows == 0) return GS_OK;
  GS_REQUIRE(out_mean && gs::aligned16(out_mean) && (!out_self || gs::aligned16(out_self)) && out_pitch % 4 == 0 &&
                 F > 0 && pitch >= ((F + 3) / 4) * 4 && out_pitch >= F,
             "gs_gather_mean_sharded: bad output / pitch");
  const int ncol4 = (int)(out_pitch / 4);
  if (gs::tuning("gather_variant", 2) != 0 && ncol4 <= 2 * 160) {
    gs::GatherImg img;
    memset(&img, 0, sizeof(img));
    return gs::launch_gather_tma2(sr, F, tab, include_self, (float*)out_self, (float*)out_mean, out_pitch, img,
                                  (cudaStream_t)stream);
  }
  int threads = ((ncol4 + 31) / 32) * 32;
  if (threads > 256) threads = 256;
  int64_t blocks = tab.total_rows;
  int64_t cap = (int64_t)gs::sm_count() * gs::tuning("gather_ctas_per_sm", 8);
  if (blocks > cap) blocks = cap;
  gs::gather_mean_sharded_kernel<5><<<(unsigned)blocks, threads, 0, (cudaStream_t)stream>>>(
      sr, F, tab, include_self, (float*)out_self, (float*)out_mean, out_pitch);
  return gs::launch_check("gather_mean_sharded_kernel");
}

int32_t gs_gather_rows_sharded(const gs_sharded_table* table_host, int32_t dtype, int32_t F, int64_t pitch,
                               const int32_t* ids, int64_t n, void* out, int64_t out_pitch, void* stream) {
  GS_REQUIRE(dtype == GS_F32, "gs_gather_rows_sharded: only GS_F32 (dtype=%d)", dtype);
  gs::ShardRows sr;
  int32_t rc = fill_shard_tab(table_host, sr, pitch, "gs_gather_rows_sharded");
  if (rc != GS_OK) return rc;
  if (n == 0) return GS_OK;
  GS_REQUIRE(ids && out && gs::aligned16(out) && out_pitch % 4 == 0 && F > 0 && pitch >= ((F + 3) / 4) * 4 && out_pitch >= F,
             "gs_gather_rows_sharded: bad arguments");
  int64_t blocks = (n + 7) / 8;
  int64_t cap = (int64_t)gs::sm_count() * 8;
  if (blocks > cap) blocks = cap;
  gs::gather_rows_sharded_kernel<<<(unsigned)blocks, 256, 0, (cudaStream_t)stream>>>(sr, F, ids, n, (float*)out, out_pitch);
  return gs::launch_check("gather_rows_sharded_kernel");
}

int32_t gs_shard_alloc(int64_t bytes, void** dev_ptr_out) {
  GS_REQUIRE(bytes > 0 && dev_ptr_out, "gs_shard_alloc: bad arguments");
  GS_CUDA(cudaMalloc(dev_ptr_out, (size_t)bytes));
  return GS_OK;
}

int32_t gs_shard_free(void* dev_ptr) {
  if (dev_ptr) GS_CUDA(cudaFree(dev_ptr));
  return GS_OK;
}

int32_t gs_ipc_export(const void* dev_ptr, uint8_t* handle64_out_host) {
  GS_REQUIRE(dev_ptr && handle64_out_host, "gs_ipc_export: NULL argument");
  static_assert(sizeof(cudaIpcMemHandle_t) == 64, "cudaIpcMemHandle_t is 64 bytes");
  cudaIpcMemHandle_t h;
  GS_CUDA(cudaIpcGetMemHandle(&h, const_cast<void*>(dev_ptr)));
  memcpy(handle64_out_host, &h, 64);
  return GS_OK;
}

int32_t gs_ipc_import(const uint8_t* handle64_host, void** dev_ptr_out) {
  GS_REQUIRE(handle64_host && dev_ptr_out, "gs_ipc_import: NULL argument");
  cudaIpcMemHandle_t h;
  memcpy(&h, handle64_host, 64);
  GS_CUDA(cudaIpcOpenMemHandle(dev_ptr_out, h, cudaIpcMemLazyEnablePeerAccess));
  return GS_OK;
}

int32_t gs_ipc_close(void* dev_ptr) {
  if (dev_ptr) GS_CUDA(cudaIpcCloseMemHandle(dev_ptr));
  return GS_OK;
}

}
```

### graphsage_b200/ops.py

```python
import torch

from . import _lib
from ._lib import (ACT_NONE, ACT_RELU, COMBINE_ADD, COMBINE_CONCAT, MATH_FP32_SIMT, MATH_TF32X3, MATH_TF32,
                   MATH_BF16, GemmPart, GemmRowIds, RowRange, Segment, check, lib, ptr, require_cuda, stream_ptr)

_U64 = 2**64 - 1

PROBE = None
LAUNCHES = 0
STAGE_HOOK = None

CACHE_EPOCH = [0]
REPACK_ALWAYS = [False]


def _probe(name):
    if STAGE_HOOK is not None:
        STAGE_HOOK(name, "pre")
    if PROBE is None:
        return _PostHook(name) if STAGE_HOOK is not None else None
    e0, e1 = torch.cuda.Event(enable_timing=True), torch.cuda.Event(enable_timing=True)
    PROBE.setdefault(name, []).append((e0, e1))
    e0.record()
    return e1


class _PostHook(object):
    def __init__(self, name):
        self.name = name

    def record(self):
        if STAGE_HOOK is not None:
            STAGE_HOOK(self.name, "post")


def _launched(n=1, ev=None):
    global LAUNCHES
    LAUNCHES += n
    if ev is not None:
        ev.record()


def pad_cols(f):
    return (int(f) + 7) // 8 * 8


def _i32(t, name):
    if t.dtype != torch.int32:
        raise TypeError("%s must be int32 (got %s)" % (name, t.dtype))
    return t.contiguous()


def sample_padded(adj, ids, k, seed, counter, col_perm=None, counter_dev=None, out=None):
    require_cuda(adj, ids, col_perm, counter_dev)
    adj, ids = _i32(adj, "adj"), _i32(ids.reshape(-1), "ids")
    n = ids.numel()
    if out is None:
        out = torch.empty((n, k), dtype=torch.int32, device=adj.device)
    ev = _probe("sample_padded")
    check(lib().gs_sample_padded(ptr(adj), adj.shape[0], adj.shape[1], ptr(ids), n, k, ptr(col_perm), seed & _U64,
                                 counter & _U64, ptr(counter_dev), ptr(out), stream_ptr()))
    _launched(1 if n * k else 0, ev)
    return out


def sample_padded_khop(adj, seeds, fanouts, seed, counter, counter_dev=None):
    require_cuda(adj, seeds, counter_dev)
    adj, seeds = _i32(adj, "adj"), _i32(seeds.reshape(-1), "seeds")
    n = seeds.numel()
    outs, cnt = [], n
    for k in fanouts:
        cnt *= int(k)
        outs.append(torch.empty((cnt,), dtype=torch.int32, device=adj.device))
    fan = (_lib.c_i32 * len(fanouts))(*[int(k) for k in fanouts])
    optr = (_lib.c_vp * len(fanouts))(*[ptr(o) for o in outs])
    ev = _probe("sample_padded_khop")
    check(lib().gs_sample_padded_khop(ptr(adj), adj.shape[0], adj.shape[1], ptr(seeds), n, fan, len(fanouts),
                                      seed & _U64, counter & _U64, ptr(counter_dev), optr, stream_ptr()))
    _launched(1 if n else 0, ev)
    return outs


def build_padded_adj(indptr, indices, max_degree, seed=123, counter=0, skip=None):
    require_cuda(indptr, indices, skip)
    if indptr.dtype != torch.int64:
        raise TypeError("indptr must be int64")
    indices = _i32(indices, "indices")
    n = indptr.numel() - 1
    adj = torch.empty((n + 1, max_degree), dtype=torch.int32, device=indptr.device)
    deg = torch.empty((n,), dtype=torch.float32, device=indptr.device)
    sk = None if skip is None else skip.to(torch.uint8).contiguous()
    check(lib().gs_build_padded_adj(ptr(indptr), ptr(indices), n, max_degree, ptr(sk), seed & _U64, counter & _U64,
                                    ptr(adj), ptr(deg), stream_ptr()))
    _launched(1)
    return adj, deg


def sample_unigram(cdf, num_sampled, seed, counter, counter_dev=None):
    require_cuda(cdf, counter_dev)
    if cdf.dtype != torch.float64:
        raise TypeError("cdf must be float64")
    out = torch.empty((num_sampled,), dtype=torch.int32, device=cdf.device)
    check(lib().gs_sample_unigram(ptr(cdf), cdf.numel(), num_sampled, seed & _U64, counter & _U64, ptr(counter_dev),
                                  ptr(out), stream_ptr()))
    _launched(1 if num_sampled else 0)
    return out


def sample_unigram_unique(cdf, num_sampled, seed, counter, counter_dev=None, status=None):
    require_cuda(cdf, counter_dev, status)
    if cdf.dtype != torch.float64:
        raise TypeError("cdf must be float64")
    if status is not None and (status.dtype != torch.int32 or status.numel() < 1):
        raise TypeError("status must be an int32 tensor with >= 1 element")
    if not 0 <= int(num_sampled) <= min(_lib.MAX_UNIQUE_SAMPLED, cdf.numel()):
        raise ValueError("num_sampled must be in [0, min(%d, %d)] (got %d)" % (_lib.MAX_UNIQUE_SAMPLED, cdf.numel(), num_sampled))
    out = torch.empty((num_sampled,), dtype=torch.int32, device=cdf.device)
    ev = _probe("sample_unigram_unique")
    check(lib().gs_sample_unigram_unique(ptr(cdf), cdf.numel(), int(num_sampled), seed & _U64, counter & _U64, ptr(counter_dev),
                                         ptr(out), ptr(status), stream_ptr()))
    _launched(1 if num_sampled else 0, ev)
    return out


def sample_csr(indptr, indices, ids, k, seed, counter, replace_if_short=True, pad_id=-1, counter_dev=None):
    require_cuda(indptr, indices, ids)
    if indptr.dtype != torch.int64:
        raise TypeError("indptr must be int64")
    indices, ids = _i32(indices, "indices"), _i32(ids.reshape(-1), "ids")
    n = ids.numel()
    out = torch.empty((n, k), dtype=torch.int32, device=ids.device)
    check(lib().gs_sample_csr(ptr(indptr), ptr(indices), indptr.numel() - 1, ptr(ids), n, k, int(bool(replace_if_short)),
                              seed & _U64, counter & _U64, ptr(counter_dev), pad_id, ptr(out), stream_ptr()))
    _launched(1 if n * k else 0)
    return out


def random_walks(indptr, indices, starts, num_walks, walk_len, seed, counter=0, start_offset=0):
    require_cuda(indptr, indices, starts)
    if indptr.dtype != torch.int64:
        raise TypeError("indptr must be int64")
    indptr, indices, starts = indptr.contiguous(), _i32(indices, "indices"), _i32(starts.reshape(-1), "starts")
    num_walks, walk_len, start_offset = int(num_walks), int(walk_len), int(start_offset)
    if not 1 <= num_walks <= _lib.WALK_MAX_WALKS:
        raise ValueError("num_walks must be in [1, %d] (got %d)" % (_lib.WALK_MAX_WALKS, num_walks))
    if not 2 <= walk_len <= _lib.WALK_MAX_LEN:
        raise ValueError("walk_len must be in [2, %d] (got %d)" % (_lib.WALK_MAX_LEN, walk_len))
    n = starts.numel()
    if not (start_offset >= 0 and start_offset + n <= 2**32):
        raise ValueError("start_offset + len(starts) must be in [0, 2^32] (got %d + %d)" % (start_offset, n))
    nbytes = lib().gs_random_walks_workspace_bytes(n, num_walks, walk_len)
    if nbytes < 0:
        check(-1)
    dev = starts.device
    ws = torch.empty((max(nbytes, 1),), dtype=torch.uint8, device=dev)
    n_pairs = torch.empty((1,), dtype=torch.int64, device=dev)
    ev = _probe("random_walks/%d" % (n * num_walks))
    check(lib().gs_random_walks(ptr(indptr), ptr(indices), indptr.numel() - 1, ptr(starts), n, num_walks, walk_len,
                                seed & _U64, counter & _U64, start_offset, ptr(ws), nbytes, ptr(n_pairs), stream_ptr()))
    out = torch.empty((int(n_pairs.item()), 2), dtype=torch.int32, device=dev)
    check(lib().gs_random_walks_emit(ptr(starts), n, num_walks, walk_len, ptr(ws), nbytes, ptr(out), stream_ptr()))
    _launched(3 if n else 0, ev)
    return out


def _dtype_code(t):
    if t.dtype == torch.float32:
        return _lib.GS_F32
    if t.dtype == torch.bfloat16:
        return _lib.GS_BF16
    raise TypeError("features must be float32 or bfloat16 (got %s)" % t.dtype)


def gather_rows(feats, ids, out=None):
    if hasattr(feats, "c_table"):
        ids = _i32(ids.reshape(-1), "ids")
        n, F = ids.numel(), feats.shape[1]
        if out is None:
            out = torch.empty((n, pad_cols(F)), dtype=torch.float32, device=feats.device)[:, :F]
        check(lib().gs_gather_rows_sharded(feats.c_table(), _lib.GS_F32, F, feats.pitch, ptr(ids), n, ptr(out),
                                           out.stride(0), stream_ptr()))
        _launched(1 if n else 0)
        return out
    require_cuda(feats, ids)
    if feats.dim() != 2 or feats.stride(1) != 1:
        raise ValueError("features must be a row-major 2-D tensor")
    ids = _i32(ids.reshape(-1), "ids")
    n, F = ids.numel(), feats.shape[1]
    if out is None:
        out = torch.empty((n, F), dtype=feats.dtype, device=feats.device)
    check(lib().gs_gather_rows(ptr(feats), _dtype_code(feats), feats.shape[0], F, feats.stride(0), ptr(ids), n,
                               ptr(out), out.stride(0), stream_ptr()))
    _launched(1 if n * F else 0)
    return out


def gather_rows_f32(feats, ids=None, row0=0, n=None, out=None):
    require_cuda(feats, ids, out)
    if feats.dim() != 2 or feats.stride(1) != 1:
        raise ValueError("features must be a row-major 2-D tensor")
    F = feats.shape[1]
    if ids is not None:
        ids = _i32(ids.reshape(-1), "ids")
        n = ids.numel() if n is None else int(n)
    if n is None:
        raise ValueError("n is required without ids")
    if out is None:
        out = torch.empty((n, pad_cols(F)), dtype=torch.float32, device=feats.device)[:, :F]
    if out.dtype != torch.float32 or out.stride(1) != 1 or out.shape[0] < n:
        raise ValueError("out must be a row-major float32 matrix with >= n rows")
    check(lib().gs_gather_rows_f32(ptr(feats), _dtype_code(feats), feats.shape[0], F, feats.stride(0), ptr(ids), int(row0), n,
                                   ptr(out), out.stride(0), stream_ptr()))
    _launched(1 if n else 0)
    return out


def cast_rows_bf16(x, out=None):
    require_cuda(x, out)
    if x.dtype != torch.float32 or x.dim() != 2 or x.stride(1) != 1:
        raise ValueError("x must be a row-major float32 matrix")
    n, F = x.shape
    if out is None:
        out = torch.empty((n, pad_cols(F)), dtype=torch.bfloat16, device=x.device)[:, :F]
    if out.dtype != torch.bfloat16 or out.stride(1) != 1 or out.shape[0] < n or out.stride(0) < F:
        raise ValueError("out must be a row-major bfloat16 matrix with >= n rows")
    check(lib().gs_cast_rows_bf16(ptr(x), n, F, x.stride(0), ptr(out), out.stride(0), stream_ptr()))
    _launched(1 if n else 0)
    return out


class Seg(object):
    __slots__ = ("n", "k", "self_ids", "neigh_ids", "self_row0", "neigh_row0", "out_row0")

    def __init__(self, n, k, self_ids=None, neigh_ids=None, self_row0=0, neigh_row0=0, out_row0=0):
        self.n, self.k = int(n), int(k)
        self.self_ids = None if self_ids is None else _i32(self_ids.reshape(-1), "self_ids")
        self.neigh_ids = None if neigh_ids is None else _i32(neigh_ids.reshape(-1), "neigh_ids")
        self.self_row0, self.neigh_row0, self.out_row0 = int(self_row0), int(neigh_row0), int(out_row0)
        if self.self_ids is not None and self.self_ids.numel() < self.n:
            raise ValueError("self_ids shorter than n")
        if self.neigh_ids is not None and self.neigh_ids.numel() < self.n * self.k:
            raise ValueError("neigh_ids shorter than n*k")

    def c_struct(self):
        require_cuda(self.self_ids, self.neigh_ids)
        return Segment(ptr(self.self_ids), ptr(self.neigh_ids), self.self_row0, self.neigh_row0, self.n, self.k, 0,
                       self.out_row0)


def make_segment(n, k, self_ids=None, neigh_ids=None, self_row0=0, neigh_row0=0, out_row0=0):
    return Seg(n, k, self_ids, neigh_ids, self_row0, neigh_row0, out_row0)



def _check_out(t, rows, out_pitch, name):
    if t is None:
        return
    require_cuda(t)
    if t.dtype != torch.float32 or t.dim() != 2 or t.stride(1) != 1 or t.stride(0) != out_pitch or t.shape[0] < rows:
        raise ValueError("%s must be a float32 [>= %d, .] CUDA matrix with row stride out_pitch = %d" % (name, rows, out_pitch))


def gather_mean(src, segments, include_self=False, want_self=True, out_pitch=None, out_mean=None, out_self=None):
    if hasattr(src, "c_table"):
        return _gather_mean_sharded(src, segments, include_self, want_self, out_pitch, out_mean, out_self)
    require_cuda(src)
    if src.dtype not in (torch.float32, torch.bfloat16) or src.dim() != 2 or src.stride(1) != 1:
        raise ValueError("src must be a row-major float32 (or bfloat16) 2-D tensor")
    F = src.shape[1]
    if out_pitch is None:
        out_pitch = pad_cols(F)
    rows = max([s.out_row0 + s.n for s in segments] + [0])
    _check_out(out_mean, rows, out_pitch, "out_mean")
    _check_out(out_self if want_self else None, rows, out_pitch, "out_self")
    if out_mean is None:
        out_mean = torch.empty((rows, out_pitch), dtype=torch.float32, device=src.device)
    if want_self and out_self is None:
        out_self = torch.empty((rows, out_pitch), dtype=torch.float32, device=src.device)
    arr = (Segment * max(len(segments), 1))(*[s.c_struct() for s in segments])
    ev = _probe("gather_mean/%d" % rows)
    check(lib().gs_gather_mean(ptr(src), _dtype_code(src), src.shape[0], F, src.stride(0), arr, len(segments),
                               int(bool(include_self)), ptr(out_self) if want_self else 0, ptr(out_mean), out_pitch,
                               stream_ptr()))
    _launched(1 if rows else 0, ev)
    return (out_self if want_self else None), out_mean


def translate_ids(table, ids):
    ids = _i32(ids.reshape(-1), "ids")
    out = torch.empty_like(ids)
    check(lib().gs_translate_ids(table.c_table(), ptr(ids), ids.numel(), ptr(out), stream_ptr()))
    _launched(1 if ids.numel() else 0)
    return out


def _shard_prepare(src, segments):
    F = src.shape[1]
    locators, staging = 0, None
    by_ids = any(s.self_ids is not None or s.neigh_ids is not None for s in segments)
    if by_ids and src.world > 1 and getattr(src, "stage_halo", True):
        lists, order = {}, []
        for s in segments:
            if s.self_ids is None or s.neigh_ids is None:
                raise ValueError("with halo staging every segment of a sharded gather must address its rows by ids")
            for t in (s.self_ids, s.neigh_ids):
                key = (t.data_ptr(), t.numel())
                if key not in lists:
                    lists[key] = t
                    order.append(key)
        capacity = sum(lists[k].numel() for k in order)
        dev = src.device
        claim = torch.empty((src.shape[0],), dtype=torch.int32, device=dev)
        count = torch.empty((1,), dtype=torch.int32, device=dev)
        stage_ids = torch.empty((capacity,), dtype=torch.int32, device=dev)
        staging = torch.empty((capacity, src.pitch), dtype=torch.float32, device=dev)
        check(lib().gs_halo_begin(ptr(claim), src.shape[0], ptr(count), stream_ptr()))
        for k in order:
            check(lib().gs_halo_claim(src.c_table(), ptr(lists[k]), lists[k].numel(), ptr(claim), ptr(count), ptr(stage_ids),
                                      capacity, stream_ptr()))
        check(lib().gs_halo_fetch(src.c_table(), F, src.pitch, ptr(stage_ids), ptr(count), capacity, ptr(staging), src.pitch,
                                  stream_ptr()))
        locs = {}
        for k in order:
            locs[k] = torch.empty_like(lists[k])
            check(lib().gs_halo_translate(src.c_table(), ptr(lists[k]), lists[k].numel(), ptr(claim), ptr(locs[k]), stream_ptr()))
        _launched(2 * len(order) + 1)
        segments = [Seg(s.n, s.k, locs[(s.self_ids.data_ptr(), s.self_ids.numel())],
                        locs[(s.neigh_ids.data_ptr(), s.neigh_ids.numel())], s.self_row0, s.neigh_row0, s.out_row0)
                    for s in segments]
        locators = 2
    elif by_ids and getattr(src, "remap", None) is not None:
        done, segs = {}, []

        def tr(t):
            key = (t.data_ptr(), t.numel())
            if key not in done:
                done[key] = translate_ids(src, t)
            return done[key]

        for s in segments:
            if s.self_ids is None or s.neigh_ids is None:
                raise ValueError("with replicas every segment of a sharded gather must address its rows by ids")
            segs.append(Seg(s.n, s.k, tr(s.self_ids), tr(s.neigh_ids), s.self_row0, s.neigh_row0, s.out_row0))
        segments, locators = segs, 1
    return segments, locators, staging


def _gather_mean_sharded(src, segments, include_self, want_self, out_pitch, out_mean, out_self):
    F = src.shape[1]
    if out_pitch is None:
        out_pitch = pad_cols(F)
    rows = max([s.out_row0 + s.n for s in segments] + [0])
    _check_out(out_mean, rows, out_pitch, "out_mean")
    _check_out(out_self if want_self else None, rows, out_pitch, "out_self")
    if out_mean is None:
        out_mean = torch.empty((rows, out_pitch), dtype=torch.float32, device=src.device)
    if want_self and out_self is None:
        out_self = torch.empty((rows, out_pitch), dtype=torch.float32, device=src.device)
    segments, locators, staging = _shard_prepare(src, segments)
    arr = (Segment * max(len(segments), 1))(*[s.c_struct() for s in segments])
    ev = _probe("gather_mean/%d" % rows)
    check(lib().gs_gather_mean_sharded(src.c_table(), _lib.GS_F32, F, src.pitch, arr, len(segments),
                                       int(bool(include_self)), locators, ptr(staging), ptr(out_self) if want_self else 0,
                                       ptr(out_mean), out_pitch, stream_ptr()))
    _launched(1 if rows else 0, ev)
    return (out_self if want_self else None), out_mean


def gather_mean_images(src, segments, include_self=False, want_self=True):
    sharded = hasattr(src, "c_table")
    if not sharded:
        require_cuda(src)
        if src.dtype != torch.float32 or src.dim() != 2 or src.stride(1) != 1:
            return None
    F = src.shape[1]
    pitch = src.pitch if sharded else src.stride(0)
    if F > 1280 or pitch % 4 != 0 or (not sharded and src.data_ptr() % 16 != 0):
        return None
    rows = max([s.out_row0 + s.n for s in segments] + [0])
    if rows == 0:
        return None
    nbytes = lib().gs_gather_mean_img_bytes(rows, F, int(bool(want_self)))
    dev = src.device
    buf = torch.empty((nbytes + 1024,), dtype=torch.uint8, device=dev)
    off = (-buf.data_ptr()) % 1024
    images = buf[off:off + nbytes]
    locators, staging = 0, None
    if sharded:
        segments, locators, staging = _shard_prepare(src, segments)
    arr = (Segment * max(len(segments), 1))(*[s.c_struct() for s in segments])
    ev = _probe("gather_mean/%d" % rows)
    rc = lib().gs_gather_mean_img(0 if sharded else ptr(src), 0 if sharded else src.shape[0], src.c_table() if sharded else None,
                                  locators, ptr(staging), F, pitch, arr, len(segments), int(bool(include_self)),
                                  int(bool(want_self)), ptr(images), stream_ptr())
    if rc == -3:
        return None
    check(rc)
    _launched(1, ev)
    return images, rows


def sage_gemm_img(M, images, parts, combine=COMBINE_ADD, bias=None, act=ACT_NONE, packed=None, a_part0=0, out=None):
    _, arr, keep = _gemm_parts([(None, K, B) for (_, K, B) in parts])
    ntot = sum(p[2].shape[1] for p in parts) if (combine == COMBINE_CONCAT) else parts[0][2].shape[1]
    dev = images.device
    if out is None:
        out = torch.empty((M, ntot), dtype=torch.float32, device=dev)
    if packed is None:
        packed = PackedWeights()
    ws = packed.get(parts, arr, MATH_TF32X3, dev)
    ev = _probe("sage_gemm/%d" % M)
    check(lib().gs_sage_gemm_img(M, arr, len(parts), combine, ptr(bias), act, ptr(out), out.stride(0), ptr(ws), ptr(images),
                                 int(a_part0), stream_ptr()))
    _launched(1 if M else 0, ev)
    return out


def segment_max(x, n, k):
    require_cuda(x)
    C = x.shape[1]
    out = torch.empty((n, C), dtype=torch.float32, device=x.device)
    check(lib().gs_segment_max(ptr(x), n, k, C, x.stride(0), ptr(out), out.stride(0), stream_ptr()))
    _launched(1 if n * C else 0)
    return out


CSR_OPS = {"mean": _lib.CSR_MEAN, "mean_self": _lib.CSR_MEAN_SELF, "max": _lib.CSR_MAX}


def csr_aggregate(src, indptr, indices, op, rows=None, out=None):
    require_cuda(src, indptr, indices, rows, out)
    if src.dtype not in (torch.float32, torch.bfloat16) or src.dim() != 2 or src.stride(1) != 1:
        raise ValueError("src must be a row-major float32 (or bfloat16) 2-D tensor")
    if indptr.dtype != torch.int64 or indptr.dim() != 1 or indptr.numel() < 1:
        raise TypeError("indptr must be a 1-D int64 tensor with >= 1 element")
    if op not in CSR_OPS:
        raise ValueError("op must be one of %s (got %r)" % (sorted(CSR_OPS), op))
    indptr, indices = indptr.contiguous(), _i32(indices.reshape(-1), "indices")
    if indices.numel() == 0:
        indices = torch.zeros((1,), dtype=torch.int32, device=indptr.device)
    n_nodes = indptr.numel() - 1
    if rows is not None:
        rows = _i32(rows.reshape(-1), "rows")
    n, F = (n_nodes + 1 if rows is None else rows.numel()), src.shape[1]
    if out is None:
        out = torch.empty((n, pad_cols(F)), dtype=torch.float32, device=src.device)
    if out.dtype != torch.float32 or out.dim() != 2 or out.stride(1) != 1 or out.shape[0] < n:
        raise ValueError("out must be a row-major float32 [>= %d, .] CUDA matrix" % n)
    ev = _probe("csr_aggregate/%d" % n)
    check(lib().gs_csr_aggregate(ptr(src), _dtype_code(src), src.shape[0], F, src.stride(0), ptr(indptr), ptr(indices),
                                 n_nodes, ptr(rows), n, CSR_OPS[op], ptr(out), out.stride(0), stream_ptr()))
    _launched(1 if n else 0, ev)
    return out[:n, :F]


class TableRows(object):
    __slots__ = ("table", "ranges", "M")

    def __init__(self, table, ranges, M):
        require_cuda(table)
        if table.dtype != torch.float32 or table.dim() != 2 or table.stride(1) != 1:
            raise ValueError("the row table must be a row-major float32 matrix")
        if len(ranges) > _lib.MAX_SEGMENTS:
            raise ValueError("at most %d id ranges" % _lib.MAX_SEGMENTS)
        self.table, self.M = table, int(M)
        self.ranges = [(_i32(ids.reshape(-1), "ids"), int(row0)) for ids, row0 in ranges]
        require_cuda(*[ids for ids, _ in self.ranges])

    @property
    def device(self):
        return self.table.device

    def c_struct(self):
        r = GemmRowIds(self.table.shape[0], len(self.ranges), 0)
        for s, (ids, row0) in enumerate(self.ranges):
            r.ranges[s] = RowRange(ptr(ids), row0, ids.numel())
        return r


def _gemm_parts(parts):
    A0 = parts[0][0]
    M = A0.M if isinstance(A0, TableRows) else (A0.shape[0] if A0 is not None else 0)
    arr = (GemmPart * len(parts))()
    keep = []
    for i, (A, K, B) in enumerate(parts):
        by_id = isinstance(A, TableRows)
        if by_id:
            if A.M != M:
                raise ValueError("bad A operand for part %d" % i)
            A = A.table
        require_cuda(A, B)
        if (A is not None and A.dtype != torch.float32) or B.dtype != torch.float32:
            raise TypeError("sage_gemm operands must be float32")
        if A is not None and (A.stride(1) != 1 or (A.shape[0] != M and not by_id) or A.shape[1] < K):
            raise ValueError("bad A operand for part %d" % i)
        B = B.contiguous()
        if B.shape[0] != K:
            raise ValueError("part %d: B has %d rows, expected K=%d" % (i, B.shape[0], K))
        keep.append(B)
        arr[i] = GemmPart(ptr(A), A.stride(0) if A is not None else K, K, ptr(B), B.stride(0), B.shape[1])
    return M, arr, keep


class PackedWeights(object):

    def __init__(self):
        self.key, self.ws = None, None

    def get(self, parts, arr, math, dev):
        if REPACK_ALWAYS[0]:
            return self._pack(parts, arr, math, dev, None)
        key = (CACHE_EPOCH[0], math) + tuple((p[2].data_ptr(), p[2]._version, tuple(p[2].shape)) for p in parts)
        if key != self.key:
            self.ws = self._pack(parts, arr, math, dev, self.ws)
            self.key = key
        return self.ws

    @staticmethod
    def _pack(parts, arr, math, dev, ws):
        nbytes = lib().gs_sage_gemm_workspace_bytes(1, arr, len(parts), math)
        if nbytes < 0:
            check(-1)
        if ws is None or ws.numel() < nbytes:
            ws = torch.empty((max(nbytes, 1),), dtype=torch.uint8, device=dev)
        check(lib().gs_sage_gemm_pack(arr, len(parts), math, ptr(ws), stream_ptr()))
        _launched(1)
        return ws


def sage_gemm(parts, combine=COMBINE_ADD, bias=None, act=ACT_NONE, math=MATH_FP32_SIMT, out=None, packed=None):
    M, arr, keep = _gemm_parts(parts)
    rid = None
    if any(isinstance(p[0], TableRows) for p in parts):
        rid = (GemmRowIds * len(parts))()
        for i, p in enumerate(parts):
            if isinstance(p[0], TableRows):
                rid[i] = p[0].c_struct()
    ntot = sum(p[2].shape[1] for p in parts) if (combine == COMBINE_CONCAT) else parts[0][2].shape[1]
    dev = parts[0][0].device
    if out is None:
        out = torch.empty((M, ntot), dtype=torch.float32, device=dev)

    def run(ws):
        if rid is None:
            return lib().gs_sage_gemm_prepacked(M, arr, len(parts), combine, ptr(bias), act, math, ptr(out), out.stride(0),
                                                ptr(ws), stream_ptr())
        return lib().gs_sage_gemm_rows(M, arr, rid, len(parts), combine, ptr(bias), act, math, ptr(out), out.stride(0),
                                       ptr(ws), stream_ptr())

    if math == MATH_FP32_SIMT or packed is None:
        ws_bytes = lib().gs_sage_gemm_workspace_bytes(M, arr, len(parts), math)
        if ws_bytes < 0:
            check(-1)
        ws = torch.empty((ws_bytes,), dtype=torch.uint8, device=dev) if ws_bytes > 0 else None
        ev = _probe("sage_gemm/%d" % M)
        if M and ws is not None:
            check(lib().gs_sage_gemm_pack(arr, len(parts), math, ptr(ws), stream_ptr()))
        check(run(ws))
        _launched((2 if ws is not None else 1) if M else 0, ev)
        return out
    ws = packed.get(parts, arr, math, dev)
    ev = _probe("sage_gemm/%d" % M)
    check(run(ws))
    _launched(1 if M else 0, ev)
    return out


SMALL_LAYER_MAX_ROWS = 2048


def sage_layer_small(src, seg, parts, combine=COMBINE_ADD, include_self=False, bias=None, act=ACT_NONE,
                     l2_normalize=False, counter_dev=None, counter_inc=0):
    require_cuda(src, bias, counter_dev)
    if src.dtype != torch.float32 or src.stride(1) != 1:
        raise ValueError("src must be row-major float32")
    _, arr, keep = _gemm_parts([(None, K, B) for (_, K, B) in parts])
    ntot = sum(p[2].shape[1] for p in parts) if (combine == COMBINE_CONCAT) else parts[0][2].shape[1]
    rows = seg.out_row0 + seg.n
    out = torch.empty((rows, ntot), dtype=torch.float32, device=src.device)
    cseg = seg.c_struct()
    ev = _probe("sage_layer_small/%d" % rows)
    check(lib().gs_sage_layer_small(ptr(src), src.shape[0], src.shape[1], src.stride(0), cseg, int(bool(include_self)),
                                    arr, len(parts), combine, ptr(bias), act, int(bool(l2_normalize)), ptr(out),
                                    out.stride(0), ptr(counter_dev), int(counter_inc), stream_ptr()))
    _launched(1 if seg.n else 0, ev)
    return out


class PackedMlpWeights(object):

    def __init__(self):
        self.key, self.ws = None, None

    def get(self, W):
        if REPACK_ALWAYS[0]:
            return self._pack(W)
        key = (CACHE_EPOCH[0], W.data_ptr(), W._version, tuple(W.shape))
        if key != self.key:
            self.ws = self._pack(W)
            self.key = key
        return self.ws

    @staticmethod
    def _pack(W):
        K, hidden = W.shape
        nbytes = lib().gs_maxpool_mlp_workspace_bytes(K, hidden)
        ws = torch.empty((nbytes,), dtype=torch.uint8, device=W.device)
        Wc = W.contiguous()
        check(lib().gs_maxpool_mlp_pack(ptr(Wc), Wc.stride(0), K, hidden, ptr(ws), stream_ptr()))
        _launched(1)
        return ws


def maxpool_mlp_fused(table, n_groups, k, W, bias, packed, row_ids=None, row0=0, K=None, out=None, pool="max"):
    require_cuda(table, W, bias, row_ids)
    if table.dtype != torch.bfloat16 or table.stride(1) != 1:
        raise TypeError("table must be row-major bfloat16")
    K = W.shape[0] if K is None else K
    hidden = W.shape[1]
    if out is None:
        out = torch.empty((n_groups, hidden), dtype=torch.float32, device=table.device)
    ws = packed.get(W)
    if row_ids is not None:
        row_ids = _i32(row_ids.reshape(-1), "row_ids")
    ev = _probe("maxpool_mlp/%d" % n_groups)
    fn = lib().gs_meanpool_mlp_fused if pool == "mean" else lib().gs_maxpool_mlp_fused
    check(fn(ptr(table), table.shape[0], K, table.stride(0), ptr(row_ids), row0, n_groups, k,
             ptr(ws), ptr(bias), hidden, ptr(out), out.stride(0), stream_ptr()))
    _launched(1 if n_groups else 0, ev)
    return out


class PackedMlpDxWeights(PackedMlpWeights):

    def __init__(self, cols):
        PackedMlpWeights.__init__(self)
        self.cols = int(cols)

    def get(self, W):
        if REPACK_ALWAYS[0]:
            return self._pack_dx(W, self.cols)
        key = (CACHE_EPOCH[0], W.data_ptr(), W._version, tuple(W.shape), self.cols)
        if key != self.key:
            self.ws = self._pack_dx(W, self.cols)
            self.key = key
        return self.ws

    @staticmethod
    def _pack_dx(W, cols):
        if not 1 <= cols <= W.shape[0]:
            raise ValueError("pool_mlp_backward_dx: cols must be in [1, %d] (the rows of Wm), got %d" % (W.shape[0], cols))
        nbytes = lib().gs_pool_mlp_dx_pack_bytes(cols, W.shape[1])
        if nbytes < 0:
            raise ValueError("pool_mlp_backward_dx: needs 1 <= cols and hidden % 128 == 0 (cols=%d hidden=%d)"
                             % (cols, W.shape[1]))
        ws = torch.empty((nbytes,), dtype=torch.uint8, device=W.device)
        Wc = W.contiguous()
        check(lib().gs_pool_mlp_dx_pack(ptr(Wc), Wc.stride(0), cols, Wc.shape[1], ptr(ws), stream_ptr()))
        _launched(1)
        return ws


def pool_mlp_backward_dp(table, n_groups, k, W, bias, packed, dhp, row_ids=None, row0=0, K=None, pool="max"):
    require_cuda(table, W, bias, row_ids, dhp)
    if table.dtype != torch.bfloat16 or table.stride(1) != 1:
        raise TypeError("table must be row-major bfloat16")
    K = W.shape[0] if K is None else K
    hidden = W.shape[1]
    if dhp.dtype != torch.float32 or dhp.dim() != 2 or dhp.stride(1) != 1 or tuple(dhp.shape) != (n_groups, hidden):
        raise ValueError("dhp must be a float32 [%d, %d] matrix with unit column stride" % (n_groups, hidden))
    nbytes = lib().gs_pool_mlp_dp_bytes(n_groups, k, hidden)
    if nbytes < 0:
        raise ValueError("pool_mlp_backward_dp: needs k <= 128 and hidden % 128 == 0 (k=%d hidden=%d)" % (k, hidden))
    grad = torch.empty((max(nbytes, 16),), dtype=torch.uint8, device=table.device)
    if row_ids is not None:
        row_ids = _i32(row_ids.reshape(-1), "row_ids")
    ws = packed.get(W)
    ev = _probe("pool_mlp_backward_dp/%d" % n_groups)
    check(lib().gs_pool_mlp_backward_dp(ptr(table), table.shape[0], K, table.stride(0), ptr(row_ids), row0, n_groups, k,
                                        ptr(ws), ptr(bias), hidden, ptr(dhp), dhp.stride(0), int(pool == "mean"), ptr(grad),
                                        stream_ptr()))
    _launched(1 if n_groups else 0, ev)
    return grad


def pool_mlp_backward_dw(table, n_groups, k, grad, dWm, dbm, row_ids=None, row0=0, K=None):
    require_cuda(table, grad, dWm, dbm, row_ids)
    K = dWm.shape[0] if K is None else K
    hidden = dWm.shape[1]
    if dWm.dtype != torch.float32 or not dWm.is_contiguous() or dbm.dtype != torch.float32 or not dbm.is_contiguous() \
            or dbm.numel() != hidden:
        raise ValueError("dWm must be a contiguous float32 [K, hidden] matrix and dbm a contiguous float32 [hidden]")
    nbytes = lib().gs_pool_mlp_dw_workspace_bytes(n_groups, k, K, hidden)
    if nbytes < 0:
        raise ValueError("pool_mlp_backward_dw: needs k <= 128 and hidden % 128 == 0 (k=%d hidden=%d)" % (k, hidden))
    ws = torch.empty((max(nbytes, 16),), dtype=torch.uint8, device=table.device)
    if row_ids is not None:
        row_ids = _i32(row_ids.reshape(-1), "row_ids")
    ev = _probe("pool_mlp_backward_dw/%d" % n_groups)
    check(lib().gs_pool_mlp_backward_dw(ptr(table), table.shape[0], K, table.stride(0), ptr(row_ids), row0, n_groups, k,
                                        hidden, ptr(grad), ptr(ws), nbytes, ptr(dWm), dWm.stride(0), ptr(dbm), stream_ptr()))
    _launched(4 if n_groups else 0, ev)
    return dWm, dbm


def pool_mlp_backward_dx(grad, n_groups, k, W, packed_dx, out=None):
    require_cuda(grad, W, out)
    cols, hidden = packed_dx.cols, W.shape[1]
    if out is None:
        out = torch.empty((n_groups * k, pad_cols(cols)), dtype=torch.float32, device=grad.device)[:, :cols]
    if out.dtype != torch.float32 or out.stride(1) != 1 or out.shape[0] < n_groups * k or out.shape[1] < cols:
        raise ValueError("out must be a row-major float32 [>= %d, >= %d] matrix" % (n_groups * k, cols))
    ws = packed_dx.get(W)
    ev = _probe("pool_mlp_backward_dx/%d" % n_groups)
    check(lib().gs_pool_mlp_backward_dx(n_groups, k, hidden, ptr(grad), ptr(ws), cols, ptr(out), out.stride(0), stream_ptr()))
    _launched(1 if n_groups else 0, ev)
    return out


def dropout_site(site):
    seed, call, rate = site[:3]
    call_dev = site[3] if len(site) > 3 else None
    rate = float(rate)
    if not 0.0 <= rate < 1.0:
        raise ValueError("dropout rate must be in [0, 1) (got %r)" % (rate,))
    if call_dev is not None:
        require_cuda(call_dev)
        if call_dev.dtype != torch.int64 or call_dev.numel() < 1:
            raise TypeError("call_dev must be an int64 CUDA tensor with >= 1 element")
    return _lib.DropoutSite(int(seed) & _U64, int(call) & 0xFFFFFFFF, rate, ptr(call_dev))


def gather_mean_dropout(src, segments, neigh_sites, self_sites, include_self=False, want_self=True, out_pitch=None):
    require_cuda(src)
    if hasattr(src, "c_table") or src.dtype != torch.float32 or src.dim() != 2 or src.stride(1) != 1:
        raise ValueError("gather_mean_dropout needs a row-major float32 CUDA table")
    if len(segments) > _lib.MAX_SEGMENTS or len(neigh_sites) != len(segments) or len(self_sites) != len(segments):
        raise ValueError("gather_mean_dropout takes at most %d segments and one neighbour and one self site per segment"
                         % _lib.MAX_SEGMENTS)
    F = src.shape[1]
    if out_pitch is None:
        out_pitch = pad_cols(F)
    rows = max([s.out_row0 + s.n for s in segments] + [0])
    out_mean = torch.empty((rows, out_pitch), dtype=torch.float32, device=src.device)
    out_self = torch.empty((rows, out_pitch), dtype=torch.float32, device=src.device) if want_self else None
    nseg = max(len(segments), 1)
    arr = (Segment * nseg)(*[s.c_struct() for s in segments])
    ns = (_lib.DropoutSite * nseg)(*[dropout_site(x) for x in neigh_sites])
    ss = (_lib.DropoutSite * nseg)(*[dropout_site(x) for x in self_sites])
    ev = _probe("gather_mean_dropout/%d" % rows)
    check(lib().gs_gather_mean_dropout(ptr(src), src.shape[0], F, src.stride(0), arr, len(segments), ns, ss,
                                       int(bool(include_self)), ptr(out_self), ptr(out_mean), out_pitch, stream_ptr()))
    _launched(1 if rows else 0, ev)
    return out_self, out_mean


def dropout_apply(x, site, rows=None, group=1, scale=1.0, out=None, accumulate=False):
    require_cuda(x, out)
    group = int(group)
    if group < 1:
        raise ValueError("group must be >= 1")
    if x.dtype != torch.float32 or x.dim() != 2 or (x.stride(1) != 1 and x.shape[1] > 1):
        raise ValueError("x must be a float32 matrix with unit column stride")
    F = x.shape[1]
    rows = x.shape[0] * group if rows is None else int(rows)
    if x.shape[0] < (rows + group - 1) // group:
        raise ValueError("x has %d rows, %d needed" % (x.shape[0], (rows + group - 1) // group))
    c_site = dropout_site(site)
    if out is None:
        if accumulate:
            raise ValueError("accumulate needs out")
        out = torch.empty((rows, F), dtype=torch.float32, device=x.device)
    if out.dtype != torch.float32 or out.dim() != 2 or out.shape[0] < rows or out.shape[1] != F \
            or (out.stride(1) != 1 and F > 1):
        raise ValueError("out must be a float32 [>= %d, %d] matrix with unit column stride" % (rows, F))
    ldx, ldo = max(x.stride(0), F), max(out.stride(0), F)
    if out.data_ptr() == x.data_ptr() and (group != 1 or ldx != ldo):
        raise ValueError("in-place dropout_apply needs group == 1 and equal row strides")
    ev = _probe("dropout_apply/%d" % rows)
    check(lib().gs_dropout_apply(ptr(x), ldx, rows, F, group, float(scale), c_site, int(bool(accumulate)), ptr(out), ldo,
                                 stream_ptr()))
    _launched(1 if rows * F else 0, ev)
    return out


def _embed_lists(lists, d, who):
    if len(lists) > _lib.MAX_EMBED_LISTS:
        raise ValueError("%s takes at most %d lists" % (who, _lib.MAX_EMBED_LISTS))
    arr = (_lib.EmbedGradList * max(len(lists), 1))()
    keep = []
    dev = None
    for i, (ids, grad, group, scale) in enumerate(lists):
        require_cuda(ids, grad)
        ids = _i32(ids.reshape(-1), "ids")
        n, group = ids.numel(), int(group)
        if group < 1:
            raise ValueError("group must be >= 1")
        if grad.dtype != torch.float32 or grad.dim() != 2 or (grad.stride(1) != 1 and grad.shape[1] > 1) \
                or grad.shape[1] < d or grad.shape[0] < (n + group - 1) // group:
            raise ValueError("list %d: grad must be a float32 [>= %d, >= %d] matrix with unit column stride"
                             % (i, (n + group - 1) // group, d))
        keep.append(ids)
        dev = grad.device
        arr[i] = _lib.EmbedGradList(ptr(ids), ptr(grad), max(grad.stride(0), d), n, group, float(scale))
    return arr, keep, dev


def embedding_grad(lists, n_rows, d, out=None, sites=None):
    if sites is not None and len(sites) != len(lists):
        raise ValueError("embedding_grad: one site per list")
    arr, keep, dev = _embed_lists(lists, d, "embedding_grad")
    if out is None:
        out = torch.empty((n_rows, d), dtype=torch.float32, device=dev if dev is not None else "cuda")
    require_cuda(out)
    if out.dtype != torch.float32 or out.dim() != 2 or out.shape[0] != n_rows or out.shape[1] != d \
            or (out.stride(1) != 1 and d > 1):
        raise ValueError("out must be a float32 [%d, %d] matrix with unit column stride" % (n_rows, d))
    nbytes = lib().gs_embedding_grad_workspace_bytes(arr, len(lists), int(n_rows), int(d))
    if nbytes < 0:
        check(-1)
    ws = torch.empty((nbytes,), dtype=torch.uint8, device=out.device) if nbytes > 0 else None
    ev = _probe("embedding_grad/%d" % sum(k.numel() for k in keep))
    if sites is None:
        check(lib().gs_embedding_grad(arr, len(lists), int(n_rows), int(d), ptr(out), max(out.stride(0), d), ptr(ws), nbytes,
                                      stream_ptr()))
    else:
        c_sites = (_lib.DropoutSite * max(len(sites), 1))(*[dropout_site(s) for s in sites])
        check(lib().gs_embedding_grad_dropout(arr, c_sites, len(lists), int(n_rows), int(d), ptr(out), max(out.stride(0), d),
                                              ptr(ws), nbytes, stream_ptr()))
    _launched(3 if nbytes > 0 and n_rows * d else 0, ev)
    return out


def _fp32_table(t, name, min_cols):
    require_cuda(t)
    if t.dtype != torch.float32 or t.dim() != 2 or (t.stride(1) != 1 and t.shape[1] > 1) or t.shape[1] < min_cols:
        raise ValueError("%s must be a float32 CUDA matrix with >= %d columns and unit column stride" % (name, min_cols))


def embedding_sgd(table, lists, lr):
    _fp32_table(table, "table", 1)
    n_rows, d = table.shape
    arr, keep, _ = _embed_lists(lists, d, "embedding_sgd")
    nbytes = lib().gs_embedding_grad_workspace_bytes(arr, len(lists), int(n_rows), int(d))
    if nbytes < 0:
        check(-1)
    ws = torch.empty((nbytes,), dtype=torch.uint8, device=table.device) if nbytes > 0 else None
    ev = _probe("embedding_sgd/%d" % sum(k.numel() for k in keep))
    check(lib().gs_embedding_sgd(arr, len(lists), int(n_rows), int(d), -float(lr), ptr(table), max(table.stride(0), d), ptr(ws),
                                 nbytes, stream_ptr()))
    _launched(3 if nbytes > 0 and n_rows * d else 0, ev)
    return table


def skipgram_grad(target, context, batch1, batch2, neg):
    _fp32_table(target, "target", 1)
    d = target.shape[1]
    _fp32_table(context, "context", d + 1)
    if context.shape[0] != target.shape[0]:
        raise ValueError("target and context must have the same number of rows")
    require_cuda(batch1, batch2, neg)
    batch1, batch2, neg = _i32(batch1.reshape(-1), "batch1"), _i32(batch2.reshape(-1), "batch2"), _i32(neg.reshape(-1), "neg")
    B, S = batch1.numel(), neg.numel()
    if batch2.numel() != B or B < 1:
        raise ValueError("batch1 and batch2 must hold the same number (>= 1) of ids")
    if not 1 <= S <= _lib.MAX_UNIQUE_SAMPLED:
        raise ValueError("the number of negatives must be in [1, %d] (got %d)" % (_lib.MAX_UNIQUE_SAMPLED, S))
    dev = target.device
    f32 = dict(dtype=torch.float32, device=dev)
    wd = pad_cols(d + 1)
    out = dict(loss=torch.empty((), **f32), aff=torch.empty((B,), **f32), neg_aff=torch.empty((B, S), **f32),
               gt=torch.empty((B, pad_cols(d)), **f32)[:, :d], gc_pos=torch.empty((B, wd), **f32)[:, :d + 1],
               gc_neg=torch.empty((S, wd), **f32)[:, :d + 1])
    nbytes = lib().gs_skipgram_workspace_bytes(B, S, d)
    if nbytes < 0:
        check(-1)
    ws = torch.empty((nbytes,), dtype=torch.uint8, device=dev)
    ev = _probe("skipgram_grad/%d" % B)
    check(lib().gs_skipgram_grad(ptr(target), target.stride(0), ptr(context), context.stride(0), target.shape[0], d, ptr(batch1),
                                 ptr(batch2), B, ptr(neg), S, ptr(out["loss"]), ptr(out["aff"]), ptr(out["neg_aff"]),
                                 ptr(out["gt"]), out["gt"].stride(0), ptr(out["gc_pos"]), ptr(out["gc_neg"]), wd, ptr(ws), nbytes,
                                 stream_ptr()))
    _launched(2, ev)
    return out


def _rows_f32(t, name, cols):
    require_cuda(t)
    if t.dtype != torch.float32 or t.dim() != 2 or t.stride(1) != 1 or t.shape[1] < cols:
        raise ValueError("%s must be a row-major float32 matrix with >= %d columns" % (name, cols))
    return t


def seq_lengths(x, n, k):
    _rows_f32(x, "x", 0)
    if x.shape[0] != n * k:
        raise ValueError("x has %d rows, expected n*k = %d" % (x.shape[0], n * k))
    out = torch.empty((n,), dtype=torch.int32, device=x.device)
    ev = _probe("seq_lengths/%d" % n)
    check(lib().gs_seq_lengths(ptr(x), x.stride(0), n, k, x.shape[1], ptr(out), stream_ptr()))
    _launched(1 if n else 0, ev)
    return out


def lstm_forward(P, Wh, lengths, n, k, out=None, train=False):
    H = Wh.shape[0]
    _rows_f32(P, "P", 4 * H)
    _rows_f32(Wh, "Wh", 4 * H)
    lengths = _i32(lengths, "lengths")
    dev = P.device
    if out is None:
        out = torch.empty((n, H), dtype=torch.float32, device=dev)
    _rows_f32(out, "out", H)
    saved = [torch.empty((n * k, w), dtype=torch.float32, device=dev) for w in (4 * H, H, H)] if train else [None] * 3
    g, c, hp = saved
    ev = _probe("lstm_forward/%d" % n)
    check(lib().gs_lstm_forward(ptr(P), P.stride(0), ptr(Wh), Wh.stride(0), ptr(lengths), n, k, H, ptr(out), out.stride(0),
                                ptr(g), 4 * H, ptr(c), H, ptr(hp), H, stream_ptr()))
    _launched(1 if n else 0, ev)
    return (out, g, c, hp) if train else out


def lstm_backward(dh_last, gates, c, lengths, Wh, n, k):
    H = Wh.shape[0]
    _rows_f32(dh_last, "dh_last", H)
    _rows_f32(gates, "gates", 4 * H)
    _rows_f32(c, "c", H)
    _rows_f32(Wh, "Wh", 4 * H)
    lengths = _i32(lengths, "lengths")
    dz = torch.empty((n * k, 4 * H), dtype=torch.float32, device=gates.device)
    ev = _probe("lstm_backward/%d" % n)
    check(lib().gs_lstm_backward(ptr(dh_last), dh_last.stride(0), ptr(gates), gates.stride(0), ptr(c), c.stride(0),
                                 ptr(lengths), ptr(Wh), Wh.stride(0), n, k, H, ptr(dz), dz.stride(0), stream_ptr()))
    _launched(1 if n else 0, ev)
    return dz


def l2_normalize_rows_(x):
    require_cuda(x)
    check(lib().gs_l2_normalize_rows(ptr(x), x.shape[0], x.shape[1], x.stride(0), stream_ptr()))
    _launched(1 if x.numel() else 0)
    return x
```

### include/graphsage_b200.h

```cpp
#ifndef GRAPHSAGE_B200_H_
#define GRAPHSAGE_B200_H_

#include <stdint.h>

#ifdef __cplusplus
extern "C" {
#endif

#define GS_ABI_VERSION 2

typedef enum {
  GS_OK = 0,
  GS_ERR_INVALID_ARG = -1,
  GS_ERR_CUDA = -2,
  GS_ERR_UNSUPPORTED = -3
} gs_status;

typedef enum { GS_F32 = 0, GS_BF16 = 1, GS_F64 = 2 } gs_dtype;
typedef enum { GS_ACT_NONE = 0, GS_ACT_RELU = 1 } gs_act;
typedef enum {
  GS_COMBINE_ADD = 0,
  GS_COMBINE_CONCAT = 1
} gs_combine;
typedef enum {
  GS_MATH_FP32_SIMT = 0,
  GS_MATH_TF32X3 = 1,
  GS_MATH_TF32 = 2,
  GS_MATH_BF16 = 3
} gs_math;

int32_t gs_version(void);
const char* gs_last_error_string(void);
int32_t gs_set_tuning(const char* key, int32_t value);

int32_t gs_sample_padded(const int32_t* adj, int64_t n_rows, int32_t max_deg,
                         const int32_t* ids, int64_t n, int32_t k,
                         const int32_t* col_perm, uint64_t seed, uint64_t counter,
                         const uint64_t* counter_dev, int32_t* out, void* stream);

#define GS_MAX_HOPS 4
int32_t gs_sample_padded_khop(const int32_t* adj, int64_t n_rows, int32_t max_deg,
                              const int32_t* seeds, int64_t n_seeds, const int32_t* fanout_host,
                              int32_t n_hops, uint64_t seed, uint64_t counter,
                              const uint64_t* counter_dev, int32_t* const* out_host, void* stream);

int32_t gs_sample_csr(const int64_t* indptr, const int32_t* indices, int64_t n_nodes,
                      const int32_t* ids, int64_t n, int32_t k, int32_t replace_if_short,
                      uint64_t seed, uint64_t counter, const uint64_t* counter_dev,
                      int32_t pad_id, int32_t* out, void* stream);

int32_t gs_sample_unigram(const double* cdf, int64_t n, int32_t num_sampled, uint64_t seed, uint64_t counter,
                          const uint64_t* counter_dev, int32_t* out, void* stream);

#define GS_MAX_UNIQUE_SAMPLED 1024
#define GS_UNIQUE_DRAW_BUDGET (1 << 20)
int32_t gs_sample_unigram_unique(const double* cdf, int64_t n, int32_t num_sampled, uint64_t seed, uint64_t counter,
                                 const uint64_t* counter_dev, int32_t* out, int32_t* status, void* stream);

int32_t gs_build_padded_adj(const int64_t* indptr, const int32_t* indices, int64_t n_nodes, int32_t max_deg,
                            const uint8_t* skip, uint64_t seed, uint64_t counter, int32_t* adj, float* deg,
                            void* stream);

int32_t gs_perm_prefix_host(uint64_t seed, uint64_t counter, int32_t max_deg, int32_t k,
                            int32_t* out_host);

int32_t gs_gather_rows(const void* feats, int32_t dtype, int64_t n_rows, int32_t F,
                       int64_t pitch, const int32_t* ids, int64_t n, void* out,
                       int64_t out_pitch, void* stream);

#define GS_MAX_SEGMENTS 4
typedef struct {
  const int32_t* self_ids;
  const int32_t* neigh_ids;
  int64_t self_row0;
  int64_t neigh_row0;
  int64_t n;
  int32_t k;
  int32_t _pad;
  int64_t out_row0;
} gs_segment;

int32_t gs_gather_mean(const void* src, int32_t dtype, int64_t n_src_rows, int32_t F, int64_t pitch,
                       const gs_segment* segments_host, int32_t n_segments, int32_t include_self,
                       void* out_self, void* out_mean, int64_t out_pitch, void* stream);

#define GS_MAX_SHARDS 16
typedef struct {
  const void* base[GS_MAX_SHARDS];
  int64_t row_start[GS_MAX_SHARDS + 1];
  int32_t n_shards;
  int32_t my_shard;
  int64_t n_global_rows;
  int64_t zero_row;
  const int32_t* remap;
} gs_sharded_table;

int32_t gs_gather_mean_sharded(const gs_sharded_table* table_host, int32_t dtype, int32_t F, int64_t pitch,
                               const gs_segment* segments_host, int32_t n_segments, int32_t include_self,
                               int32_t ids_are_locators, const void* staging, void* out_self, void* out_mean,
                               int64_t out_pitch, void* stream);
int32_t gs_halo_begin(int32_t* claim, int64_t n_global_rows, int32_t* count, void* stream);
int32_t gs_halo_claim(const gs_sharded_table* table_host, const int32_t* ids, int64_t n, int32_t* claim, int32_t* count,
                      int32_t* stage_ids, int64_t capacity, void* stream);
int32_t gs_halo_fetch(const gs_sharded_table* table_host, int32_t F, int64_t pitch, const int32_t* stage_ids,
                      const int32_t* count, int64_t capacity, float* staging, int64_t staging_pitch, void* stream);
int32_t gs_halo_translate(const gs_sharded_table* table_host, const int32_t* ids, int64_t n, const int32_t* claim,
                          int32_t* out, void* stream);
int32_t gs_translate_ids(const gs_sharded_table* table_host, const int32_t* ids, int64_t n, int32_t* out, void* stream);
int32_t gs_gather_rows_sharded(const gs_sharded_table* table_host, int32_t dtype, int32_t F, int64_t pitch,
                               const int32_t* ids, int64_t n, void* out, int64_t out_pitch, void* stream);

int32_t gs_shard_alloc(int64_t bytes, void** dev_ptr_out);
int32_t gs_shard_free(void* dev_ptr);
int32_t gs_ipc_export(const void* dev_ptr, uint8_t* handle64_out_host);
int32_t gs_ipc_import(const uint8_t* handle64_host, void** dev_ptr_out);
int32_t gs_ipc_close(void* dev_ptr);

int32_t gs_gather_rows_f32(const void* feats, int32_t dtype, int64_t n_rows, int32_t F, int64_t pitch,
                           const int32_t* ids, int64_t row0, int64_t n, float* out, int64_t out_pitch,
                           void* stream);
int32_t gs_cast_rows_bf16(const float* x, int64_t n, int32_t F, int64_t ldx, void* out_bf16, int64_t out_pitch,
                          void* stream);

int32_t gs_rmat_degrees(int32_t scale, int64_t n_nodes, double edge_factor, double a, double b, double c, double d,
                        uint64_t seed, uint64_t mul, uint64_t mul_inv, uint64_t add, int32_t* deg_out, void* stream);
int32_t gs_rmat_fill(int32_t scale, int64_t n_nodes, double a, double b, double c, double d, uint64_t seed, uint64_t mul,
                     uint64_t mul_inv, uint64_t add, const int64_t* indptr, int32_t* indices, const int64_t* long_rows,
                     int64_t n_long, int64_t long_threshold, void* stream);

int32_t gs_segment_max(const float* x, int64_t n, int32_t k, int32_t C, int64_t ldx,
                       float* out, int64_t ldo, void* stream);

typedef struct {
  const float* A; int64_t lda; int32_t K;
  const float* B; int64_t ldb; int32_t N;
} gs_gemm_part;

int64_t gs_sage_gemm_workspace_bytes(int64_t M, const gs_gemm_part* parts_host, int32_t n_parts,
                                     int32_t math);
int32_t gs_sage_gemm(int64_t M, const gs_gemm_part* parts_host, int32_t n_parts, int32_t combine,
                     const float* bias, int32_t act, int32_t math, float* out, int64_t ldo,
                     void* workspace, void* stream);

int32_t gs_sage_gemm_pack(const gs_gemm_part* parts_host, int32_t n_parts, int32_t math, void* workspace,
                          void* stream);
int32_t gs_sage_gemm_prepacked(int64_t M, const gs_gemm_part* parts_host, int32_t n_parts, int32_t combine,
                               const float* bias, int32_t act, int32_t math, float* out, int64_t ldo,
                               const void* workspace, void* stream);

typedef struct {
  const int32_t* ids;
  int64_t row0;
  int64_t n;
} gs_row_range;
typedef struct {
  int64_t n_table_rows;
  int32_t n_ranges;
  int32_t _pad;
  gs_row_range ranges[GS_MAX_SEGMENTS];
} gs_gemm_row_ids;
int32_t gs_sage_gemm_rows(int64_t M, const gs_gemm_part* parts_host, const gs_gemm_row_ids* row_ids_host, int32_t n_parts,
                          int32_t combine, const float* bias, int32_t act, int32_t math, float* out, int64_t ldo,
                          const void* workspace, void* stream);

int64_t gs_gather_mean_img_bytes(int64_t rows, int32_t F, int32_t want_self);
int32_t gs_gather_mean_img(const void* src, int64_t n_src_rows, const gs_sharded_table* table_host, int32_t ids_are_locators,
                           const void* staging, int32_t F, int64_t pitch, const gs_segment* segments_host,
                           int32_t n_segments, int32_t include_self, int32_t want_self, void* images, void* stream);
int32_t gs_sage_gemm_img(int64_t M, const gs_gemm_part* parts_host, int32_t n_parts, int32_t combine, const float* bias,
                         int32_t act, float* out, int64_t ldo, const void* workspace, const void* a_images,
                         int32_t a_part0, void* stream);

int32_t gs_sage_layer_small(const float* src, int64_t n_src_rows, int32_t F, int64_t pitch,
                            const gs_segment* segment_host, int32_t include_self,
                            const gs_gemm_part* parts_host, int32_t n_parts, int32_t combine,
                            const float* bias, int32_t act, int32_t l2_normalize,
                            float* out, int64_t ldo, uint64_t* counter_dev, uint64_t counter_inc,
                            void* stream);

int64_t gs_maxpool_mlp_workspace_bytes(int32_t K, int32_t hidden);
int32_t gs_maxpool_mlp_pack(const float* Wm, int64_t ldw, int32_t K, int32_t hidden, void* workspace,
                            void* stream);
int32_t gs_maxpool_mlp_fused(const void* table_bf16, int64_t n_rows, int32_t K, int64_t pitch,
                             const int32_t* row_ids, int64_t row0, int64_t n_groups, int32_t k,
                             const void* packed_weights, const float* bias, int32_t hidden,
                             float* out, int64_t ldo, void* stream);
int32_t gs_meanpool_mlp_fused(const void* table_bf16, int64_t n_rows, int32_t K, int64_t pitch,
                              const int32_t* row_ids, int64_t row0, int64_t n_groups, int32_t k,
                              const void* packed_weights, const float* bias, int32_t hidden,
                              float* out, int64_t ldo, void* stream);

int64_t gs_pool_mlp_dp_bytes(int64_t n_groups, int32_t k, int32_t hidden);
int32_t gs_pool_mlp_backward_dp(const void* table_bf16, int64_t n_rows, int32_t K, int64_t pitch,
                                const int32_t* row_ids, int64_t row0, int64_t n_groups, int32_t k,
                                const void* packed_weights, const float* bias, int32_t hidden, const float* dhp,
                                int64_t lddhp, int32_t pool_mean, void* dp, void* stream);
int64_t gs_pool_mlp_dw_workspace_bytes(int64_t n_groups, int32_t k, int32_t K, int32_t hidden);
int32_t gs_pool_mlp_backward_dw(const void* table_bf16, int64_t n_rows, int32_t K, int64_t pitch,
                                const int32_t* row_ids, int64_t row0, int64_t n_groups, int32_t k, int32_t hidden,
                                const void* dp, void* workspace, int64_t workspace_bytes, float* dWm, int64_t ldw,
                                float* dbm, void* stream);
int64_t gs_pool_mlp_dx_pack_bytes(int32_t Kd, int32_t hidden);
int32_t gs_pool_mlp_dx_pack(const float* Wm, int64_t ldw, int32_t Kd, int32_t hidden, void* packed, void* stream);
int32_t gs_pool_mlp_backward_dx(int64_t n_groups, int32_t k, int32_t hidden, const void* dp, const void* packed,
                                int32_t Kd, float* dx, int64_t ldx, void* stream);

int32_t gs_pipeline_step(const void* ids_host, void* ids_dev, int64_t ids_bytes, void* const* graph_execs_host,
                         int32_t n_graphs, const void* out_dev, void* out_host, int64_t out_bytes,
                         void* h2d_stream, void* compute_stream, void* copy_stream, void* ev_ids, void* ev_done,
                         void* ev_drained);

int32_t gs_bump_counter(uint64_t* counter_dev, uint64_t inc, void* stream);

#define GS_MAX_EMBED_LISTS 8
typedef struct {
  const int32_t* ids;
  const float* grad;
  int64_t ldg;
  int64_t n;
  int32_t group;
  float scale;
} gs_embed_grad_list;

int64_t gs_embedding_grad_workspace_bytes(const gs_embed_grad_list* lists_host, int32_t n_lists, int64_t n_rows,
                                          int32_t d);
int32_t gs_embedding_grad(const gs_embed_grad_list* lists_host, int32_t n_lists, int64_t n_rows, int32_t d, float* out,
                          int64_t ldo, void* workspace, int64_t workspace_bytes, void* stream);

typedef struct {
  uint64_t seed;
  uint32_t call;
  float rate;
  const uint64_t* call_dev;
} gs_dropout_site;

int32_t gs_gather_mean_dropout(const float* src, int64_t n_src_rows, int32_t F, int64_t pitch, const gs_segment* segments_host,
                               int32_t n_segments, const gs_dropout_site* neigh_sites_host,
                               const gs_dropout_site* self_sites_host, int32_t include_self, float* out_self,
                               float* out_mean, int64_t out_pitch, void* stream);

int32_t gs_dropout_apply(const float* x, int64_t ldx, int64_t rows, int32_t F, int32_t group, float scale,
                         gs_dropout_site site, int32_t accumulate, float* out, int64_t ldo, void* stream);

int32_t gs_embedding_grad_dropout(const gs_embed_grad_list* lists_host, const gs_dropout_site* sites_host, int32_t n_lists,
                                  int64_t n_rows, int32_t d, float* out, int64_t ldo, void* workspace,
                                  int64_t workspace_bytes, void* stream);

int32_t gs_embedding_sgd(const gs_embed_grad_list* lists_host, int32_t n_lists, int64_t n_rows, int32_t d, float alpha,
                         float* table, int64_t ldt, void* workspace, int64_t workspace_bytes, void* stream);

int64_t gs_skipgram_workspace_bytes(int64_t B, int32_t S, int32_t d);
int32_t gs_skipgram_grad(const float* target, int64_t ldt, const float* context, int64_t ldc, int64_t n_rows, int32_t d,
                         const int32_t* batch1, const int32_t* batch2, int64_t B, const int32_t* neg, int32_t S, float* loss,
                         float* aff, float* neg_aff, float* gt, int64_t ldgt, float* gc_pos, float* gc_neg, int64_t ldgc,
                         void* workspace, int64_t workspace_bytes, void* stream);

int32_t gs_seq_lengths(const float* x, int64_t ldx, int64_t n, int32_t k, int32_t K, int32_t* len, void* stream);
int32_t gs_lstm_forward(const float* P, int64_t ldp, const float* Wh, int64_t ldw, const int32_t* len, int64_t n, int32_t k,
                        int32_t H, float* h_last, int64_t ldh, float* gates, int64_t ldg, float* c, int64_t ldc,
                        float* h_prev, int64_t ldhp, void* stream);
int32_t gs_lstm_backward(const float* dh_last, int64_t lddh, const float* gates, int64_t ldg, const float* c, int64_t ldc,
                         const int32_t* len, const float* Wh, int64_t ldw, int64_t n, int32_t k, int32_t H, float* dZ,
                         int64_t ldz, void* stream);

#define GS_SGD_MAX_D 1024
#define GS_SGD_MAX_PROBLEMS 65535
#define GS_SGD_MAX_EPOCHS 1024
int32_t gs_sgd_orders(const uint32_t* seeds, int32_t P, int64_t n, int32_t epochs, int32_t* orders, void* stream);
int32_t gs_sgd_fit(const void* x, int32_t dtype, int64_t n, int32_t d, int64_t ldx, const int32_t* labels, int64_t ldy,
                   const int32_t* orders, int32_t P, int32_t epochs, double alpha, double optimal_init, double* coef,
                   int64_t ldc, double* intercept, void* stream);

#define GS_WALK_MAX_WALKS (1 << 20)
#define GS_WALK_MAX_LEN 33
int64_t gs_random_walks_workspace_bytes(int64_t n, int32_t num_walks, int32_t walk_len);
int32_t gs_random_walks(const int64_t* indptr, const int32_t* indices, int64_t n_nodes, const int32_t* starts, int64_t n,
                        int32_t num_walks, int32_t walk_len, uint64_t seed, uint64_t counter, int64_t start_offset,
                        void* workspace, int64_t workspace_bytes, int64_t* n_pairs, void* stream);
int32_t gs_random_walks_emit(const int32_t* starts, int64_t n, int32_t num_walks, int32_t walk_len, const void* workspace,
                             int64_t workspace_bytes, int32_t* out, void* stream);

typedef enum { GS_CSR_MEAN = 0, GS_CSR_MEAN_SELF = 1, GS_CSR_MAX = 2 } gs_csr_op;
int32_t gs_csr_aggregate(const void* src, int32_t dtype, int64_t n_src_rows, int32_t F, int64_t pitch,
                         const int64_t* indptr, const int32_t* indices, int64_t n_nodes,
                         const int32_t* rows , int64_t n, int32_t op,
                         float* out, int64_t out_pitch, void* stream);

int32_t gs_l2_normalize_rows(float* x, int64_t n, int32_t C, int64_t ldx, void* stream);

#ifdef __cplusplus
}
#endif
#endif
```

Baseline: 3.414 million.

## Use dynamic work-stealing slots in TMA gather-mean kernel with persistent CTAs

Reworks the TMA double-buffered gather-mean kernel so that each CTA holds several independent slots (sub-groups of threads with their own ring buffers, mbarriers and named barriers). Each slot claims output rows dynamically from a global atomic counter instead of a static grid stride. The grid is capped near three quarters of the SM count, and a per-call device workspace word is threaded through the APIs and zeroed with a memset. The aim is to balance load across variable-degree rows and keep more TMA loads in flight per SM. In exchange it adds an atomic per row, an extra memset launch, and a small tensor allocation per call.

```diff
diff --git a/graphsage_b200/_lib.py b/graphsage_b200/_lib.py
--- a/graphsage_b200/_lib.py
+++ b/graphsage_b200/_lib.py
@@ -27,7 +27,8 @@
 
 class ShardedTable(ctypes.Structure):
     _fields_ = [("base", c_vp * MAX_SHARDS), ("row_start", c_i64 * (MAX_SHARDS + 1)), ("n_shards", c_i32),
-                ("my_shard", c_i32), ("n_global_rows", c_i64), ("zero_row", c_i64), ("remap", c_vp)]
+                ("my_shard", c_i32), ("n_global_rows", c_i64), ("zero_row", c_i64), ("remap", c_vp),
+                ("work_counter", c_vp)]
 
 
 class GemmPart(ctypes.Structure):
@@ -71,7 +72,7 @@
     "gs_perm_prefix_host": (c_i32, [c_u64, c_u64, c_i32, c_i32, ctypes.POINTER(c_i32)]),
     "gs_gather_rows": (c_i32, [c_vp, c_i32, c_i64, c_i32, c_i64, c_vp, c_i64, c_vp, c_i64, c_vp]),
     "gs_gather_mean": (c_i32, [c_vp, c_i32, c_i64, c_i32, c_i64, ctypes.POINTER(Segment), c_i32, c_i32, c_vp, c_vp,
-                               c_i64, c_vp]),
+                               c_i64, c_vp, c_vp]),
     "gs_gather_mean_sharded": (c_i32, [ctypes.POINTER(ShardedTable), c_i32, c_i32, c_i64, ctypes.POINTER(Segment), c_i32,
                                        c_i32, c_i32, c_vp, c_vp, c_vp, c_i64, c_vp]),
     "gs_halo_begin": (c_i32, [c_vp, c_i64, c_vp, c_vp]),
@@ -129,7 +130,7 @@
     "gs_embedding_grad_workspace_bytes": (c_i64, [ctypes.POINTER(EmbedGradList), c_i32, c_i64, c_i32]),
     "gs_embedding_grad": (c_i32, [ctypes.POINTER(EmbedGradList), c_i32, c_i64, c_i32, c_vp, c_i64, c_vp, c_i64, c_vp]),
     "gs_gather_mean_dropout": (c_i32, [c_vp, c_i64, c_i32, c_i64, ctypes.POINTER(Segment), c_i32, ctypes.POINTER(DropoutSite),
-                                       ctypes.POINTER(DropoutSite), c_i32, c_vp, c_vp, c_i64, c_vp]),
+                                       ctypes.POINTER(DropoutSite), c_i32, c_vp, c_vp, c_i64, c_vp, c_vp]),
     "gs_dropout_apply": (c_i32, [c_vp, c_i64, c_i64, c_i32, c_i32, ctypes.c_float, DropoutSite, c_i32, c_vp, c_i64, c_vp]),
     "gs_embedding_grad_dropout": (c_i32, [ctypes.POINTER(EmbedGradList), ctypes.POINTER(DropoutSite), c_i32, c_i64, c_i32, c_vp,
                                           c_i64, c_vp, c_i64, c_vp]),
diff --git a/graphsage_b200/csrc/gather.cu b/graphsage_b200/csrc/gather.cu
--- a/graphsage_b200/csrc/gather.cu
+++ b/graphsage_b200/csrc/gather.cu
@@ -1,3 +1,5 @@
+#include <algorithm>
+
 #include "common.cuh"
 
 namespace gs {
@@ -236,6 +238,7 @@
 };
 
 constexpr int kGroupRows = 13;
+constexpr int64_t kImgCounterBytes = 128;
 
 struct GatherImg {
   unsigned char* base;
@@ -258,20 +261,31 @@
   *reinterpret_cast<uint4*>(dst + 16384) = lo;
 }
 
+constexpr int kGatherMaxSlots = 8;
+constexpr int kGatherMaxThreads = 640;
+
 template <class Rows, bool kDrop>
-__global__ void __launch_bounds__(192, 3) gather_mean_tma2_kernel(const __grid_constant__ Rows rows_of, int F,
-                                                               const __grid_constant__ SegTable tab,
-                                                               int include_self, float* __restrict__ out_self,
-                                                               float* __restrict__ out_mean, int64_t out_pitch,
-                                                               int row_bytes, const __grid_constant__ GatherImg img,
-                                                               const __grid_constant__ DropTab drop) {
+__global__ void __launch_bounds__(kGatherMaxThreads, 1) gather_mean_tma2_kernel(const __grid_constant__ Rows rows_of, int F,
+                                                                                const __grid_constant__ SegTable tab,
+                                                                                int include_self, float* __restrict__ out_self,
+                                                                                float* __restrict__ out_mean, int64_t out_pitch,
+                                                                                int row_bytes, int slot_threads,
+                                                                                unsigned long long* __restrict__ work_counter,
+                                                                                const __grid_constant__ GatherImg img,
+                                                                                const __grid_constant__ DropTab drop) {
   extern __shared__ __align__(128) unsigned char smem[];
-  __shared__ __align__(8) uint64_t bar[2];
+  __shared__ __align__(8) uint64_t bars[kGatherMaxSlots][2];
+  __shared__ int64_t claimed[kGatherMaxSlots][2];
   __shared__ uint32_t drop_off[2 * GS_MAX_SEGMENTS];
-  if (threadIdx.x == 0) {
+  const int slot = threadIdx.x / slot_threads;
+  const int tid = threadIdx.x - slot * slot_threads;
+  const uint32_t bar_id = 1u + (uint32_t)slot;
+  uint64_t* bar = bars[slot];
+  if (tid == 0) {
     mbar_init(&bar[0], 1);
     mbar_init(&bar[1], 1);
     fence_mbar_init();
+    claimed[slot][0] = (int64_t)atomicAdd(work_counter, 1ull);
   }
   if constexpr (kDrop) {
     if (threadIdx.x < 2 * GS_MAX_SEGMENTS) {
@@ -280,14 +294,22 @@
     }
   }
   __syncthreads();
+  auto slot_sync = [&]() { asm volatile("bar.sync %0, %1;" ::"r"(bar_id), "r"(slot_threads) : "memory"); };
   const int ncol4 = (int)(out_pitch >> 2);
   const int row_f4 = row_bytes >> 4;
   const size_t buf_bytes = (size_t)kGroupRows * row_bytes;
+  unsigned char* ring = smem + (size_t)slot * 2 * buf_bytes;
   const int self_rows = (include_self || out_self || (img.base && img.want_self)) ? 1 : 0;
 
-  int64_t r_issue = blockIdx.x;
+  int64_t r_issue = claimed[slot][0];
   int g_issue = 0;
-  auto issue = [&](int buf) -> bool {
+  int cell = 0;
+  bool reload = false;
+  auto issue = [&](int buf, int64_t& r_out, int& g_out) -> bool {
+    if (reload) {
+      r_issue = *reinterpret_cast<volatile int64_t*>(&claimed[slot][cell]);
+      reload = false;
+    }
     if (r_issue >= tab.total_rows) return false;
     int64_t i;
     const gs_segment& sg = tab.s[find_segment(tab, r_issue, i)];
@@ -295,30 +317,43 @@
     const int rows_total = k + self_rows;
     const int first = g_issue * kGroupRows;
     const int cnt = min(kGroupRows, rows_total - first);
-    if (threadIdx.x < 32) {
-      if (threadIdx.x == 0) mbar_expect_tx(&bar[buf], (uint32_t)(cnt * row_bytes));
+    const bool last = first + cnt >= rows_total;
+    if (tid < 32) {
+      if (tid == 0) mbar_expect_tx(&bar[buf], (uint32_t)(cnt * row_bytes));
       __syncwarp();
-      for (int j = threadIdx.x; j < cnt; j += 32) {
+      for (int j = tid; j < cnt; j += 32) {
         const int jj = first + j;
         int64_t id;
         if (jj < k) id = sg.neigh_ids ? (int64_t)sg.neigh_ids[i * k + jj] : sg.neigh_row0 + i * k + jj;
         else id = sg.self_ids ? (int64_t)sg.self_ids[i] : sg.self_row0 + i;
-        bulk_g2s(smem + buf * buf_bytes + (size_t)j * row_bytes, rows_of.row(id), (uint32_t)row_bytes, &bar[buf]);
+        bulk_g2s(ring + buf * buf_bytes + (size_t)j * row_bytes, rows_of.row(id), (uint32_t)row_bytes, &bar[buf]);
       }
     }
-    if (first + cnt >= rows_total) { r_issue += gridDim.x; g_issue = 0; } else { ++g_issue; }
+    r_out = r_issue;
+    g_out = g_issue;
+    if (last) {
+      cell ^= 1;
+      if (tid == 0) claimed[slot][cell] = (int64_t)atomicAdd(work_counter, 1ull);
+      reload = true;
+      g_issue = 0;
+    } else {
+      ++g_issue;
+    }
     return true;
   };
 
   uint32_t phase[2] = {0u, 0u};
   int buf = 0;
-  bool have = issue(0);
-  int64_t r = blockIdx.x;
+  int64_t r = 0;
   int g = 0;
+  bool have = issue(0, r, g);
+  slot_sync();
   float4 acc[2];
   acc[0] = acc[1] = make_float4(0.f, 0.f, 0.f, 0.f);
   while (have) {
-    const bool have_next = issue(buf ^ 1);
+    int64_t r_next = 0;
+    int g_next = 0;
+    const bool have_next = issue(buf ^ 1, r_next, g_next);
     int64_t i;
     const int si = find_segment(tab, r, i);
     const gs_segment& sg = tab.s[si];
@@ -329,13 +364,13 @@
     const bool last = first + cnt >= rows_total;
     mbar_wait(&bar[buf], phase[buf]);
     phase[buf] ^= 1u;
-    const float4* rows = reinterpret_cast<const float4*>(smem + buf * buf_bytes);
+    const float4* rows = reinterpret_cast<const float4*>(ring + buf * buf_bytes);
     const int nn = last ? cnt - self_rows : cnt;
     DropSite nsite{};
     if constexpr (kDrop) nsite = with_call_offset(drop.neigh[si], drop_off[si]);
 #pragma unroll
     for (int q = 0; q < 2; ++q) {
-      const int c = threadIdx.x + q * blockDim.x;
+      const int c = tid + q * slot_threads;
       if (c < ncol4 && c * 4 < F) {
         float4 a = acc[q];
         for (int j = 0; j < nn; ++j) {
@@ -351,7 +386,7 @@
       const int ncol_img = img.base ? img.kblocks * 8 : 0;
 #pragma unroll
       for (int q = 0; q < 2; ++q) {
-        const int c = threadIdx.x + q * blockDim.x;
+        const int c = tid + q * slot_threads;
         if (c < ncol4 || c < ncol_img) {
           float4 a = make_float4(0.f, 0.f, 0.f, 0.f), sv = a;
           if (c < ncol4 && c * 4 < F) {
@@ -377,14 +412,12 @@
           if (c < ncol4) acc[q] = make_float4(0.f, 0.f, 0.f, 0.f);
         }
       }
-      r += gridDim.x;
-      g = 0;
-    } else {
-      ++g;
-    }
-    __syncthreads();
+    }
+    slot_sync();
     buf ^= 1;
     have = have_next;
+    r = r_next;
+    g = g_next;
   }
 }
 
@@ -832,27 +865,31 @@
 namespace gs {
 template <class Rows, bool kDrop = false>
 static int32_t launch_gather_tma2(const Rows& rows_of, int F, const SegTable& tab, int include_self, float* out_self, float* out_mean,
-                                  int64_t out_pitch, const GatherImg& img, cudaStream_t st, const DropTab* drop = nullptr) {
-  const int32_t rc_attr = ensure_dyn_smem((const void*)gather_mean_tma2_kernel<Rows, kDrop>, 200 * 1024);
+                                  int64_t out_pitch, const GatherImg& img, void* work_counter, cudaStream_t st,
+                                  const DropTab* drop = nullptr) {
+  GS_REQUIRE(work_counter && (reinterpret_cast<uintptr_t>(work_counter) & 7u) == 0,
+             "gather_mean: the work counter must be an 8-byte aligned device word");
+  constexpr int kDynSmem = 226 * 1024;
+  const int32_t rc_attr = ensure_dyn_smem((const void*)gather_mean_tma2_kernel<Rows, kDrop>, kDynSmem);
   if (rc_attr != GS_OK) return rc_attr;
   const int ncol4 = (int)(out_pitch / 4);
   const int row_bytes = ((F + 3) / 4) * 16;
-  const size_t smem2 = (size_t)2 * kGroupRows * row_bytes;
+  const size_t ring_bytes = (size_t)2 * kGroupRows * row_bytes;
   int threads = ((ncol4 + 31) / 32) * 32;
   if (threads > 160) threads = 160;
   if (threads < 32) threads = 32;
-  int per_sm = (int)((224 * 1024) / (smem2 + 1024));
-  if (per_sm < 1) per_sm = 1;
-  int lim = tuning("gather_ctas_per_sm", 8);
-  if (per_sm > lim) per_sm = lim;
-  int64_t blocks = tab.total_rows;
-  int64_t cap = (int64_t)sm_count() * per_sm;
-  if (blocks > cap) blocks = cap;
+  int slots = (int)(kDynSmem / ring_bytes);
+  slots = std::min(slots, std::min(kGatherMaxSlots, kGatherMaxThreads / threads));
+  GS_REQUIRE(slots >= 1, "gather_mean: a %zu-byte ring does not fit in shared memory", ring_bytes);
+  int64_t blocks = std::min<int64_t>(tab.total_rows, (3 * sm_count() + 3) / 4);
+  const int cap = tuning("gather_sms", 0);
+  if (cap > 0 && blocks > cap) blocks = cap;
   DropTab no_drop;
   memset(&no_drop, 0, sizeof(no_drop));
-  gather_mean_tma2_kernel<Rows, kDrop><<<(unsigned)blocks, threads, smem2, st>>>(rows_of, F, tab, include_self, out_self,
-                                                                                 out_mean, out_pitch, row_bytes, img,
-                                                                                 drop ? *drop : no_drop);
+  GS_CUDA(cudaMemsetAsync(work_counter, 0, sizeof(unsigned long long), st));
+  gather_mean_tma2_kernel<Rows, kDrop><<<(unsigned)blocks, threads * slots, ring_bytes * slots, st>>>(
+      rows_of, F, tab, include_self, out_self, out_mean, out_pitch, row_bytes, threads,
+      reinterpret_cast<unsigned long long*>(work_counter), img, drop ? *drop : no_drop);
   return launch_check("gather_mean_tma2_kernel");
 }
 }
@@ -901,7 +938,7 @@
 
 int32_t gs_gather_mean(const void* src, int32_t dtype, int64_t n_src_rows, int32_t F, int64_t pitch,
                        const gs_segment* segments_host, int32_t n_segments, int32_t include_self, void* out_self,
-                       void* out_mean, int64_t out_pitch, void* stream) {
+                       void* out_mean, int64_t out_pitch, void* workspace, void* stream) {
   GS_REQUIRE(dtype == GS_F32 || dtype == GS_BF16, "gs_gather_mean: dtype %d (GS_F32 or GS_BF16)", dtype);
   GS_REQUIRE(n_segments >= 0 && n_segments <= GS_MAX_SEGMENTS, "gs_gather_mean: n_segments=%d (max %d)", n_segments,
              GS_MAX_SEGMENTS);
@@ -970,7 +1007,8 @@
     const gs::DenseRows rows_of{fsrc, n_src_rows, pitch};
     gs::GatherImg img;
     memset(&img, 0, sizeof(img));
-    return gs::launch_gather_tma2(rows_of, F, tab, include_self, (float*)out_self, (float*)out_mean, out_pitch, img, st);
+    return gs::launch_gather_tma2(rows_of, F, tab, include_self, (float*)out_self, (float*)out_mean, out_pitch, img, workspace,
+                                  st);
   }
   if (variant >= 1 && smem <= 200 * 1024) {
     {
@@ -1067,7 +1105,7 @@
 int32_t gs_gather_mean_dropout(const float* src, int64_t n_src_rows, int32_t F, int64_t pitch, const gs_segment* segments_host,
                                int32_t n_segments, const gs_dropout_site* neigh_sites_host,
                                const gs_dropout_site* self_sites_host, int32_t include_self, float* out_self,
-                               float* out_mean, int64_t out_pitch, void* stream) {
+                               float* out_mean, int64_t out_pitch, void* workspace, void* stream) {
   GS_REQUIRE(n_segments >= 0 && n_segments <= GS_MAX_SEGMENTS, "gs_gather_mean_dropout: n_segments=%d (max %d)", n_segments,
              GS_MAX_SEGMENTS);
   GS_REQUIRE((segments_host && neigh_sites_host && self_sites_host) || n_segments == 0,
@@ -1099,8 +1137,8 @@
     const gs::DenseRows rows_of{src, n_src_rows, pitch};
     gs::GatherImg img;
     memset(&img, 0, sizeof(img));
-    return gs::launch_gather_tma2<gs::DenseRows, true>(rows_of, F, tab, include_self, out_self, out_mean, out_pitch, img, st,
-                                                       &drop);
+    return gs::launch_gather_tma2<gs::DenseRows, true>(rows_of, F, tab, include_self, out_self, out_mean, out_pitch, img,
+                                                       workspace, st, &drop);
   }
   int64_t blocks = tab.total_rows;
   int64_t cap = (int64_t)gs::sm_count() * 8;
@@ -1188,7 +1226,7 @@
 int64_t gs_gather_mean_img_bytes(int64_t rows, int32_t F, int32_t want_self) {
   if (rows < 0 || F < 1) return -1;
   const int64_t n_mtiles = (rows + 127) / 128, kblocks = (F + 31) / 32;
-  return (want_self ? 2 : 1) * n_mtiles * kblocks * 2 * 16384;
+  return (want_self ? 2 : 1) * n_mtiles * kblocks * 2 * 16384 + gs::kImgCounterBytes;
 }
 
 int32_t gs_gather_mean_img(const void* src, int64_t n_src_rows, const gs_sharded_table* table_host, int32_t ids_are_locators,
@@ -1221,10 +1259,11 @@
   img.kblocks = (F + 31) / 32;
   img.n_mtiles = (int32_t)((rows + 127) / 128);
   img.want_self = want_self ? 1 : 0;
+  void* counter = (unsigned char*)images + (gs_gather_mean_img_bytes(rows, F, want_self) - gs::kImgCounterBytes);
   if (src) {
     GS_REQUIRE(gs::aligned16(src) && n_src_rows > 0, "gs_gather_mean_img: table must be 16-byte aligned");
     const gs::DenseRows rows_of{(const float*)src, n_src_rows, pitch};
-    return gs::launch_gather_tma2(rows_of, F, tab, include_self, nullptr, nullptr, out_pitch, img, (cudaStream_t)stream);
+    return gs::launch_gather_tma2(rows_of, F, tab, include_self, nullptr, nullptr, out_pitch, img, counter, (cudaStream_t)stream);
   }
   gs::ShardRows sr;
   int32_t rc = fill_shard_tab(table_host, sr, pitch, "gs_gather_mean_img");
@@ -1233,7 +1272,7 @@
              "gs_gather_mean_img: ids_are_locators = 2 needs the staging buffer");
   sr.locators = ids_are_locators;
   sr.staging = (const float*)staging;
-  return gs::launch_gather_tma2(sr, F, tab, include_self, nullptr, nullptr, out_pitch, img, (cudaStream_t)stream);
+  return gs::launch_gather_tma2(sr, F, tab, include_self, nullptr, nullptr, out_pitch, img, counter, (cudaStream_t)stream);
 }
 
 int32_t gs_halo_begin(int32_t* claim, int64_t n_global_rows, int32_t* count, void* stream) {
@@ -1323,7 +1362,7 @@
     gs::GatherImg img;
     memset(&img, 0, sizeof(img));
     return gs::launch_gather_tma2(sr, F, tab, include_self, (float*)out_self, (float*)out_mean, out_pitch, img,
-                                  (cudaStream_t)stream);
+                                  table_host->work_counter, (cudaStream_t)stream);
   }
   int threads = ((ncol4 + 31) / 32) * 32;
   if (threads > 256) threads = 256;
diff --git a/graphsage_b200/ops.py b/graphsage_b200/ops.py
--- a/graphsage_b200/ops.py
+++ b/graphsage_b200/ops.py
@@ -1,3 +1,5 @@
+import ctypes
+
 import torch
 
 from . import _lib
@@ -261,6 +263,17 @@
         raise ValueError("%s must be a float32 [>= %d, .] CUDA matrix with row stride out_pitch = %d" % (name, rows, out_pitch))
 
 
+def _gather_workspace(device):
+    return torch.empty((1,), dtype=torch.int64, device=device)
+
+
+def _table_for_call(src, workspace):
+    t = _lib.ShardedTable()
+    ctypes.memmove(ctypes.byref(t), src.c_table(), ctypes.sizeof(t))
+    t.work_counter = ptr(workspace)
+    return ctypes.byref(t), t
+
+
 def gather_mean(src, segments, include_self=False, want_self=True, out_pitch=None, out_mean=None, out_self=None):
     if hasattr(src, "c_table"):
         return _gather_mean_sharded(src, segments, include_self, want_self, out_pitch, out_mean, out_self)
@@ -278,10 +291,11 @@
     if want_self and out_self is None:
         out_self = torch.empty((rows, out_pitch), dtype=torch.float32, device=src.device)
     arr = (Segment * max(len(segments), 1))(*[s.c_struct() for s in segments])
+    ws = _gather_workspace(src.device)
     ev = _probe("gather_mean/%d" % rows)
     check(lib().gs_gather_mean(ptr(src), _dtype_code(src), src.shape[0], F, src.stride(0), arr, len(segments),
                                int(bool(include_self)), ptr(out_self) if want_self else 0, ptr(out_mean), out_pitch,
-                               stream_ptr()))
+                               ptr(ws), stream_ptr()))
     _launched(1 if rows else 0, ev)
     return (out_self if want_self else None), out_mean
 
@@ -359,8 +373,10 @@
         out_self = torch.empty((rows, out_pitch), dtype=torch.float32, device=src.device)
     segments, locators, staging = _shard_prepare(src, segments)
     arr = (Segment * max(len(segments), 1))(*[s.c_struct() for s in segments])
+    ws = _gather_workspace(src.device)
+    table, _keep = _table_for_call(src, ws)
     ev = _probe("gather_mean/%d" % rows)
-    check(lib().gs_gather_mean_sharded(src.c_table(), _lib.GS_F32, F, src.pitch, arr, len(segments),
+    check(lib().gs_gather_mean_sharded(table, _lib.GS_F32, F, src.pitch, arr, len(segments),
                                        int(bool(include_self)), locators, ptr(staging), ptr(out_self) if want_self else 0,
                                        ptr(out_mean), out_pitch, stream_ptr()))
     _launched(1 if rows else 0, ev)
@@ -748,9 +764,11 @@
     arr = (Segment * nseg)(*[s.c_struct() for s in segments])
     ns = (_lib.DropoutSite * nseg)(*[dropout_site(x) for x in neigh_sites])
     ss = (_lib.DropoutSite * nseg)(*[dropout_site(x) for x in self_sites])
+    ws = _gather_workspace(src.device)
     ev = _probe("gather_mean_dropout/%d" % rows)
     check(lib().gs_gather_mean_dropout(ptr(src), src.shape[0], F, src.stride(0), arr, len(segments), ns, ss,
-                                       int(bool(include_self)), ptr(out_self), ptr(out_mean), out_pitch, stream_ptr()))
+                                       int(bool(include_self)), ptr(out_self), ptr(out_mean), out_pitch, ptr(ws),
+                                       stream_ptr()))
     _launched(1 if rows else 0, ev)
     return out_self, out_mean
 
diff --git a/include/graphsage_b200.h b/include/graphsage_b200.h
--- a/include/graphsage_b200.h
+++ b/include/graphsage_b200.h
@@ -69,6 +69,7 @@
                        int64_t out_pitch, void* stream);
 
 #define GS_MAX_SEGMENTS 4
+#define GS_GATHER_WORKSPACE_BYTES 8
 typedef struct {
   const int32_t* self_ids;
   const int32_t* neigh_ids;
@@ -82,7 +83,7 @@
 
 int32_t gs_gather_mean(const void* src, int32_t dtype, int64_t n_src_rows, int32_t F, int64_t pitch,
                        const gs_segment* segments_host, int32_t n_segments, int32_t include_self,
-                       void* out_self, void* out_mean, int64_t out_pitch, void* stream);
+                       void* out_self, void* out_mean, int64_t out_pitch, void* workspace, void* stream);
 
 #define GS_MAX_SHARDS 16
 typedef struct {
@@ -93,6 +94,7 @@
   int64_t n_global_rows;
   int64_t zero_row;
   const int32_t* remap;
+  void* work_counter;
 } gs_sharded_table;
 
 int32_t gs_gather_mean_sharded(const gs_sharded_table* table_host, int32_t dtype, int32_t F, int64_t pitch,
@@ -237,7 +239,7 @@
 int32_t gs_gather_mean_dropout(const float* src, int64_t n_src_rows, int32_t F, int64_t pitch, const gs_segment* segments_host,
                                int32_t n_segments, const gs_dropout_site* neigh_sites_host,
                                const gs_dropout_site* self_sites_host, int32_t include_self, float* out_self,
-                               float* out_mean, int64_t out_pitch, void* stream);
+                               float* out_mean, int64_t out_pitch, void* workspace, void* stream);
 
 int32_t gs_dropout_apply(const float* x, int64_t ldx, int64_t rows, int32_t F, int32_t group, float scale,
                          gs_dropout_site site, int32_t accumulate, float* out, int64_t ldo, void* stream);
```

Result: no change. 3.394 million (median of 6 runs) (-0.6%).
